# leejaeyong7/tiny-cuda-nn

Hardware: AMD Instinct MI355X
Metric: training_step throughput (samples/s) HashGrid+64-wide FFMLP, batch=256k; % fp16-MFMA peak (higher is better)
Workload: dtype f16

## Files before the change

tiny-cuda-nn_amd/csrc/capi.cpp:

```cpp
#include "../../include/tcnn_amd.h"

#include "model.h"

#include <mutex>
#include <string>

using namespace tcnn_amd;

namespace {
thread_local std::string g_last_error;
tcnn_amd::Switches g_switches;
std::mutex g_switches_mutex;

bool env_is(const char* name, char c) {
	const char* e = getenv(name);
	return e && e[0] == c;
}
int env_01(const char* name) {
	const char* e = getenv(name);
	return (e && (e[0] == '0' || e[0] == '1')) ? e[0] - '0' : -1;
}

template <typename F>
int guarded(F&& f) {
	try {
		f();
		return TCNN_OK;
	} catch (const std::exception& e) {
		g_last_error = e.what();
		log_message(TCNN_LOG_ERROR, g_last_error);
		return TCNN_ERROR;
	} catch (...) {
		g_last_error = "unknown error";
		return TCNN_ERROR;
	}
}

Json parse_or_empty(const char* text) {
	if (!text || !*text) return Json::object();
	return Json::parse(text);
}
}

struct tcnn_module_s {
	std::unique_ptr<Model> model;
	std::string hyperparams_text;
	std::string name_text;
};

struct tcnn_context_s {
	std::unique_ptr<ModelContext> ctx;
};

struct tcnn_trainer_s {
	std::unique_ptr<Trainer> trainer;
	std::string hyperparams_text;
	std::string network_hyperparams_text;
	std::vector<uint8_t> snapshot;
};

struct tcnn_train_ctx_s {
	std::unique_ptr<TrainContext> ctx;
};

struct tcnn_optimizer_s {
	std::unique_ptr<Optimizer> optimizer;
	size_t n_params = 0;
	std::string hyperparams_text;
	std::vector<uint8_t> snapshot;
};

namespace tcnn_amd {
Switches switches() {
	std::lock_guard<std::mutex> lock{g_switches_mutex};
	return g_switches;
}
void switches_reload() {
	Switches w;
	w.grid_planes = !env_is("TCNN_AMD_GRID_PLANES", '0');
	w.grid_rows_planes = !env_is("TCNN_AMD_GRID_ROWS_PLANES", '0');
	{ const char* e = getenv("TCNN_AMD_GRID_SCATTER"); w.grid_scatter_lds = !(e && std::string{e} == "atomic"); }
	w.scatter_records = !env_is("TCNN_AMD_SCATTER_RECORDS", '0');
	w.scatter_tune = !env_is("TCNN_AMD_SCATTER_TUNE", '0');
	w.scatter_lists = env_01("TCNN_AMD_SCATTER_LISTS");
	w.scatter_wide = env_is("TCNN_AMD_SCATTER_WIDE", '1');
	w.fused_step = !env_is("TCNN_AMD_FUSED_STEP", '0');
	w.side_jobs = !env_is("TCNN_AMD_SIDE_JOBS", '0');
	w.live_image = !env_is("TCNN_AMD_LIVE_IMAGE", '0');
	w.adam_steps32 = env_is("TCNN_AMD_ADAM_STEPS32", '1');
	w.adam_in_reduce = !env_is("TCNN_AMD_ADAM_IN_REDUCE", '0');
	w.adam_prologue = !env_is("TCNN_AMD_ADAM_PROLOGUE", '0');
	w.adam_prologue_refused = env_is("TCNN_AMD_ADAM_PROLOGUE", 'r');
	w.mlp_r32 = !env_is("TCNN_AMD_MLP_R32", '0');
	w.mlp_r32a = env_01("TCNN_AMD_MLP_R32A");
	w.mlp_regs = !env_is("TCNN_AMD_MLP_REGS", '0');
	w.mlp_fast = !env_is("TCNN_AMD_MLP_FAST", '0');
	if (const char* e = getenv("TCNN_AMD_MLP_PRIO")) w.mlp_prio = (uint32_t)atoi(e);
	w.listgrad_in_mlp = !env_is("TCNN_AMD_LISTGRAD_IN_MLP", '0');
	w.mlp_layerwise = env_is("TCNN_AMD_MLP_LAYERWISE", '1');
	std::lock_guard<std::mutex> lock{g_switches_mutex};
	g_switches = w;
}
}

extern "C" {

const char* tcnn_last_error(void) { return g_last_error.c_str(); }
const char* tcnn_version(void) { return "tcnn_amd 0.1 (gfx950)"; }

uint32_t tcnn_batch_size_granularity(void) { return BATCH_SIZE_GRANULARITY; }

int tcnn_device(int* device_out) {
	return guarded([&] { HIP_CHECK_THROW(hipGetDevice(device_out)); });
}

int tcnn_set_device(int device) {
	return guarded([&] { HIP_CHECK_THROW(hipSetDevice(device)); });
}

void tcnn_free_temporary_memory(void) { Arena::instance().release_all(); }

int tcnn_gpu_malloc(size_t bytes, void** out) {
	return guarded([&] {
		CHECK_THROW(out != nullptr);
		*out = nullptr;
		if (bytes) HIP_CHECK_THROW(hipMalloc(out, bytes));
	});
}
int tcnn_gpu_free(void* ptr) {
	return guarded([&] { if (ptr) HIP_CHECK_THROW(hipFree(ptr)); });
}
int tcnn_gpu_memcpy(void* dst, const void* src, size_t bytes, int kind) {
	return guarded([&] {
		const hipMemcpyKind k = kind == TCNN_MEMCPY_HOST_TO_DEVICE ? hipMemcpyHostToDevice : kind == TCNN_MEMCPY_DEVICE_TO_HOST ? hipMemcpyDeviceToHost : hipMemcpyDeviceToDevice;
		if (bytes) HIP_CHECK_THROW(hipMemcpy(dst, src, bytes, k));
	});
}
int tcnn_gpu_memset(void* ptr, int value, size_t bytes) {
	return guarded([&] { if (bytes) HIP_CHECK_THROW(hipMemset(ptr, value, bytes)); });
}
int tcnn_stream_synchronize(tcnn_stream_t stream) {
	return guarded([&] { HIP_CHECK_THROW(hipStreamSynchronize((hipStream_t)stream)); });
}
int tcnn_generate_random_uniform(tcnn_stream_t stream, uint64_t rng_state_inc[2], size_t n, float* out, float lower, float upper) {
	return guarded([&] {
		CHECK_THROW(rng_state_inc != nullptr && (out != nullptr || n == 0));
		generate_random_uniform((hipStream_t)stream, rng_state_inc, n, out, lower, upper);
		HIP_CHECK_THROW(hipGetLastError());
	});
}
int tcnn_has_networks(void) { return 1; }
float tcnn_default_loss_scale(int precision) { return precision == TCNN_PRECISION_FP32 ? 1.0f : LOSS_SCALE_FP16; }
int tcnn_preferred_precision(void) { return TCNN_PRECISION_FP16; }

void tcnn_set_log_callback(void (*callback)(int, const char*, void*), void* user) {
	log_sink().callback = callback;
	log_sink().user = user;
}

int tcnn_create_network_with_input_encoding_precision(uint32_t n_input_dims, uint32_t n_output_dims, const char* encoding_json, const char* network_json, int precision, tcnn_module_t* out) {
	switches_reload();
	return guarded([&] {
		CHECK_THROW(out != nullptr);
		if (precision != TCNN_PRECISION_FP32 && precision != TCNN_PRECISION_FP16) throw std::runtime_error{"Unknown precision " + std::to_string(precision)};
		auto m = std::make_unique<tcnn_module_s>();
		m->model.reset(new NetworkWithInputEncoding{n_input_dims, n_output_dims, parse_or_empty(encoding_json), parse_or_empty(network_json),
		                                            precision == TCNN_PRECISION_FP32 ? Precision::Fp32 : Precision::Fp16});
		*out = m.release();
	});
}

int tcnn_create_network_with_input_encoding(uint32_t n_input_dims, uint32_t n_output_dims, const char* encoding_json, const char* network_json, tcnn_module_t* out) {
	return tcnn_create_network_with_input_encoding_precision(n_input_dims, n_output_dims, encoding_json, network_json, TCNN_PRECISION_FP16, out);
}

int tcnn_create_network_precision(uint32_t n_input_dims, uint32_t n_output_dims, const char* network_json, int precision, tcnn_module_t* out) {
	return tcnn_create_network_with_input_encoding_precision(n_input_dims, n_output_dims, "{\"otype\": \"Identity\"}", network_json, precision, out);
}

int tcnn_create_network(uint32_t n_input_dims, uint32_t n_output_dims, const char* network_json, tcnn_module_t* out) {
	return tcnn_create_network_precision(n_input_dims, n_output_dims, network_json, TCNN_PRECISION_FP16, out);
}

int tcnn_create_encoding(uint32_t n_input_dims, const char* encoding_json, int precision, tcnn_module_t* out) {
	switches_reload();
	return guarded([&] {
		CHECK_THROW(out != nullptr);
		auto m = std::make_unique<tcnn_module_s>();
		m->model.reset(new EncodingModel{n_input_dims, parse_or_empty(encoding_json), precision == TCNN_PRECISION_FP32 ? Precision::Fp32 : Precision::Fp16});
		*out = m.release();
	});
}

void tcnn_module_destroy(tcnn_module_t module) { delete module; }

int tcnn_module_inference(tcnn_module_t m, tcnn_stream_t stream, uint32_t n, const float* input, void* output, void* params) {
	return guarded([&] {
		CHECK_THROW(m && m->model);
		m->model->inference((hipStream_t)stream, n, MatView{input, m->model->input_width(), 1u}, output, params);
	});
}

int tcnn_module_forward(tcnn_module_t m, tcnn_stream_t stream, uint32_t n, const float* input, void* output, void* params, int prepare_input_gradients, tcnn_context_t* ctx_out) {
	return guarded([&] {
		CHECK_THROW(m && m->model && ctx_out);
		auto c = std::make_unique<tcnn_context_s>();
		c->ctx = m->model->forward((hipStream_t)stream, n, MatView{input, m->model->input_width(), 1u}, output, params, prepare_input_gradients != 0);
		*ctx_out = c.release();
	});
}

int tcnn_module_backward(tcnn_module_t m, tcnn_stream_t stream, tcnn_context_t ctx, uint32_t n, float* dL_dinput, const void* dL_doutput, void* dL_dparams,
                         const float* input, const void* output, const void* params) {
	return guarded([&] {
		CHECK_THROW(m && m->model);
		if (!ctx || !ctx->ctx) throw std::runtime_error{"Module::bwd: called with invalid context. fwd likely (mistakenly) ran in inference mode."};
		MatViewMut dx{dL_dinput, m->model->input_width(), 1u};
		m->model->backward((hipStream_t)stream, *ctx->ctx, n, MatView{input, m->model->input_width(), 1u}, output, dL_doutput, dL_dinput ? &dx : nullptr, params,
		                   dL_dparams, dL_dparams ? GradientMode::Overwrite : GradientMode::Ignore);
	});
}

int tcnn_module_backward_backward_input(tcnn_module_t m, tcnn_stream_t stream, tcnn_context_t ctx, uint32_t n, const float* dL_ddLdinput, const float* input, const void* dL_doutput,
                                        void* dL_dparams, void* dL_ddLdoutput, float* dL_dinput, const void* params) {
	return tcnn_module_backward_backward_input_mode(m, stream, ctx, n, dL_ddLdinput, input, dL_doutput, dL_dparams, dL_ddLdoutput, dL_dinput, params,
	                                                dL_dparams ? TCNN_GRADIENT_OVERWRITE : TCNN_GRADIENT_IGNORE);
}

int tcnn_module_backward_backward_input_mode(tcnn_module_t m, tcnn_stream_t stream, tcnn_context_t ctx, uint32_t n, const float* dL_ddLdinput, const float* input, const void* dL_doutput,
                                             void* dL_dparams, void* dL_ddLdoutput, float* dL_dinput, const void* params, int gradient_mode) {
	return guarded([&] {
		CHECK_THROW(gradient_mode == TCNN_GRADIENT_IGNORE || ((gradient_mode == TCNN_GRADIENT_OVERWRITE || gradient_mode == TCNN_GRADIENT_ACCUMULATE) && dL_dparams != nullptr));
		CHECK_THROW(m && m->model);
		if (!ctx || !ctx->ctx) throw std::runtime_error{"Module::bwd_bwd_input: called with invalid context. fwd likely (mistakenly) ran in inference mode."};
		CHECK_THROW(dL_ddLdinput != nullptr && input != nullptr);
		const uint32_t w = m->model->input_width();
		MatViewMut dx{dL_dinput, w, 1u};
		m->model->backward_backward_input((hipStream_t)stream, *ctx->ctx, n, MatView{input, w, 1u}, MatView{dL_ddLdinput, w, 1u}, dL_doutput, dL_ddLdoutput, dL_dinput ? &dx : nullptr, params,
		                                  gradient_mode == TCNN_GRADIENT_IGNORE ? nullptr : dL_dparams, (GradientMode)gradient_mode);
	});
}

void tcnn_context_destroy(tcnn_context_t ctx) { delete ctx; }

uint32_t tcnn_module_n_input_dims(tcnn_module_t m) { return m->model->input_width(); }
uint32_t tcnn_module_n_output_dims(tcnn_module_t m) { return m->model->padded_output_width(); }
size_t tcnn_module_n_params(tcnn_module_t m) { return m->model->n_params(); }
size_t tcnn_module_list_scatters(tcnn_module_t m) { return (size_t)m->model->list_scatters(); }

namespace {
[[noreturn]] void no_grid(Model& model) {
	throw std::runtime_error{"max_level: " + model.name() + " has no grid encoding (GridEncoding::set_max_level, grid_interface.h:101-123)"};
}
}

int tcnn_module_set_max_level(tcnn_module_t m, float max_level) {
	return guarded([&] {
		CHECK_THROW(m && m->model);
		if (!m->model->set_max_level(max_level)) no_grid(*m->model);
	});
}
int tcnn_module_set_max_level_gpu(tcnn_module_t m, const float* per_sample) {
	return guarded([&] {
		CHECK_THROW(m && m->model);
		if (!m->model->set_max_level_gpu(per_sample)) no_grid(*m->model);
	});
}
float tcnn_module_max_level(tcnn_module_t m) {
	float v = std::numeric_limits<float>::quiet_NaN();
	const float* per_sample = nullptr;
	guarded([&] {
		CHECK_THROW(m && m->model);
		if (!m->model->get_max_level(v, per_sample)) no_grid(*m->model);
		g_last_error.clear();
	});
	return v;
}
int tcnn_module_param_precision(tcnn_module_t m) { return (int)m->model->precision(); }
int tcnn_module_output_precision(tcnn_module_t m) { return (int)m->model->precision(); }

int tcnn_module_initialize_params(tcnn_module_t m, uint64_t seed, float* params_full_precision, float scale) {
	return guarded([&] {
		CHECK_THROW(m && m->model);
		Pcg32 rng{seed};
		m->model->initialize_params(rng, params_full_precision, scale);
		HIP_CHECK_THROW(hipDeviceSynchronize());
	});
}

const char* tcnn_module_hyperparams(tcnn_module_t m) {
	m->hyperparams_text = m->model->hyperparams().dump();
	return m->hyperparams_text.c_str();
}

const char* tcnn_module_name(tcnn_module_t m) {
	m->name_text = m->model->name();
	return m->name_text.c_str();
}

int tcnn_create_from_config_precision(uint32_t n_input_dims, uint32_t n_output_dims, const char* config_json, uint32_t seed, int precision, tcnn_trainer_t* out) {
	switches_reload();
	return guarded([&] {
		CHECK_THROW(out != nullptr);
		if (precision != TCNN_PRECISION_FP32 && precision != TCNN_PRECISION_FP16) throw std::runtime_error{"Unknown precision " + std::to_string(precision)};
		auto t = std::make_unique<tcnn_trainer_s>();
		t->trainer.reset(new Trainer{n_input_dims, n_output_dims, parse_or_empty(config_json), seed, precision == TCNN_PRECISION_FP32 ? Precision::Fp32 : Precision::Fp16});
		*out = t.release();
	});
}

int tcnn_create_from_config_seeded(uint32_t n_input_dims, uint32_t n_output_dims, const char* config_json, uint32_t seed, tcnn_trainer_t* out) {
	return tcnn_create_from_config_precision(n_input_dims, n_output_dims, config_json, seed, TCNN_PRECISION_FP16, out);
}

int tcnn_trainer_precision(tcnn_trainer_t t) {
	int v = -1;
	guarded([&] { CHECK_THROW(t && t->trainer); v = (int)t->trainer->precision(); });
	return v;
}

int tcnn_create_from_config(uint32_t n_input_dims, uint32_t n_output_dims, const char* config_json, tcnn_trainer_t* out) {
	return tcnn_create_from_config_seeded(n_input_dims, n_output_dims, config_json, 1337, out);
}

void tcnn_trainer_destroy(tcnn_trainer_t t) { delete t; }

int tcnn_trainer_training_step(tcnn_trainer_t t, tcnn_stream_t stream, uint32_t n, const float* input, int input_layout, const float* target, const float* data_pdf,
                               int run_optimizer, float* dL_dinput, int use_inference_params, int gradient_mode, const void* external_dL_dy, tcnn_train_ctx_t* ctx_out) {
	return guarded([&] {
		CHECK_THROW(t && t->trainer && ctx_out);
		Trainer& tr = *t->trainer;
		const uint32_t w = tr.model().input_width();
		MatViewMut dx = make_view_mut(dL_dinput, w, n, input_layout);
		auto c = std::make_unique<tcnn_train_ctx_s>();
		c->ctx = tr.training_step((hipStream_t)stream, n, make_view(input, w, n, input_layout), target, data_pdf, run_optimizer != 0, dL_dinput ? &dx : nullptr,
		                          use_inference_params != 0, (GradientMode)gradient_mode, external_dL_dy);
		*ctx_out = c.release();
	});
}

int tcnn_trainer_loss(tcnn_trainer_t t, tcnn_stream_t stream, tcnn_train_ctx_t ctx, float* loss_out) {
	return guarded([&] {
		CHECK_THROW(t && t->trainer && ctx && ctx->ctx && loss_out);
		*loss_out = t->trainer->loss((hipStream_t)stream, *ctx->ctx);
	});
}

int tcnn_trainer_forward(tcnn_trainer_t t, tcnn_stream_t stream, float loss_scale, uint32_t n, const float* input, int input_layout, const float* target, const float* data_pdf,
                         int use_inference_params, int prepare_input_gradients, const void* external_dL_dy, tcnn_train_ctx_t* ctx_out) {
	return guarded([&] {
		CHECK_THROW(t && t->trainer && ctx_out);
		Trainer& tr = *t->trainer;
		auto c = std::make_unique<tcnn_train_ctx_s>();
		c->ctx = tr.forward((hipStream_t)stream, loss_scale, n, make_view(input, tr.model().input_width(), n, input_layout), target, data_pdf, use_inference_params != 0,
		                    prepare_input_gradients != 0, external_dL_dy);
		*ctx_out = c.release();
	});
}

int tcnn_trainer_backward(tcnn_trainer_t t, tcnn_stream_t stream, tcnn_train_ctx_t ctx, uint32_t n, const float* input, int input_layout, float* dL_dinput,
                          int use_inference_params, int gradient_mode) {
	return guarded([&] {
		CHECK_THROW(t && t->trainer && ctx && ctx->ctx);
		Trainer& tr = *t->trainer;
		const uint32_t w = tr.model().input_width();
		MatViewMut dx = make_view_mut(dL_dinput, w, n, input_layout);
		tr.backward((hipStream_t)stream, *ctx->ctx, n, make_view(input, w, n, input_layout), dL_dinput ? &dx : nullptr, use_inference_params != 0, (GradientMode)gradient_mode);
	});
}

int tcnn_trainer_optimizer_step(tcnn_trainer_t t, tcnn_stream_t stream, float loss_scale) {
	return guarded([&] {
		CHECK_THROW(t && t->trainer);
		t->trainer->optimizer_step((hipStream_t)stream, loss_scale);
	});
}

void tcnn_train_ctx_destroy(tcnn_train_ctx_t ctx) { delete ctx; }
const void* tcnn_train_ctx_output(tcnn_train_ctx_t ctx) { return ctx->ctx->output.data(); }
const void* tcnn_train_ctx_dL_doutput(tcnn_train_ctx_t ctx) {
	if (guarded([&] { ctx->ctx->materialize(); }) != 0) return nullptr;
	return ctx->ctx->dL_doutput_ptr;
}
const float* tcnn_train_ctx_L(tcnn_train_ctx_t ctx) {
	if (guarded([&] { ctx->ctx->materialize(); }) != 0) return nullptr;
	return ctx->ctx->L.as<float>();
}

int tcnn_trainer_inference(tcnn_trainer_t t, tcnn_stream_t stream, uint32_t n, const float* input, int input_layout, float* output, int output_layout, int use_inference_params) {
	return guarded([&] {
		CHECK_THROW(t && t->trainer);
		Trainer& tr = *t->trainer;
		tr.inference((hipStream_t)stream, n, make_view(input, tr.model().input_width(), n, input_layout), make_view_mut(output, tr.model().output_width(), n, output_layout),
		             use_inference_params != 0);
	});
}

int tcnn_trainer_inference_mixed_precision(tcnn_trainer_t t, tcnn_stream_t stream, uint32_t n, const float* input, int input_layout, void* output_half, int use_inference_params) {
	return guarded([&] {
		CHECK_THROW(t && t->trainer && (output_half || n == 0));
		Trainer& tr = *t->trainer;
		tr.inference_mixed_precision((hipStream_t)stream, n, make_view(input, tr.model().input_width(), n, input_layout), output_half, use_inference_params != 0);
// ... 232 lines not shown
```

tiny-cuda-nn_amd/csrc/grid_device.h:

```cpp
#pragma once

#include "tcnn_common.h"

#include <hip/hip_fp16.h>

namespace tcnn_amd {
namespace {

typedef _Float16 half_t;

template <typename T, int N> struct VecOf { typedef T type __attribute__((ext_vector_type(N))); };
template <typename T> struct VecOf<T, 1> { typedef T type; };

__device__ inline float smoothstep(float v) { return v * v * (3.0f - 2.0f * v); }
__device__ inline float smoothstep_derivative(float v) { return 6 * v * (1.0f - v); }

__device__ inline uint32_t pos_fract(float input, float scale, uint32_t interpolation, float* pos, float* pos_derivative) {
	float p = fmaf(scale, input, 0.5f);
	const float tmp = floorf(p);
	const uint32_t cell = (uint32_t)(int)tmp;
	p -= tmp;
	if (interpolation == (uint32_t)InterpolationType::Smoothstep) {
		*pos_derivative = smoothstep_derivative(p);
		*pos = smoothstep(p);
	} else {
		*pos_derivative = 1.0f;
		*pos = p;
	}
	return cell;
}

__device__ inline uint32_t rng_hash_device(const uint32_t* pos, int n_dims) {
	const uint64_t MULT = 0x5851f42d4c957f2dULL;
	const uint32_t bits_per_dim = 64 / n_dims;
	uint64_t step = 0;
	for (int i = 0; i < n_dims; ++i) step ^= (uint64_t)pos[i] << (i * bits_per_dim);
	uint64_t inc = (1ull << 1u) | 1u;
	uint64_t state = 0;
	state = state * MULT + inc;
	state += 1337ull;
	state = state * MULT + inc;
	uint64_t cur_mult = MULT, cur_plus = inc, acc_mult = 1u, acc_plus = 0u;
	uint64_t delta = step;
	while (delta > 0) {
		if (delta & 1) {
			acc_mult *= cur_mult;
			acc_plus = acc_plus * cur_mult + cur_plus;
		}
		cur_plus = (cur_mult + 1) * cur_plus;
		cur_mult *= cur_mult;
		delta /= 2;
	}
	state = acc_mult * state + acc_plus;
	const uint64_t old = state;
	const uint32_t xorshifted = (uint32_t)(((old >> 18u) ^ old) >> 27u);
	const uint32_t rot = (uint32_t)(old >> 59u);
	return (xorshifted >> rot) | (xorshifted << ((~rot + 1u) & 31));
}

template <int D, bool RNG = true>
__device__ inline uint32_t level_index(const GridLevel& lv, const uint32_t* primes, uint32_t hash_type, const uint32_t* cell) {
	uint32_t index;
	if (lv.hashed) {
		if (RNG && hash_type == (uint32_t)HashType::Rng) {
			index = rng_hash_device(cell, D);
		} else {
			index = 0;
#pragma unroll
			for (int d = 0; d < D; ++d) index ^= cell[d] * primes[d];
		}
	} else {
		index = 0;
#pragma unroll
		for (int d = 0; d < D; ++d) index += cell[d] * lv.stride[d];
	}
	if (lv.size_mask) return index & lv.size_mask;
	return index >= lv.size ? index % lv.size : index;
}

template <int D>
__device__ inline void load_coords(const MatView& x, uint32_t i, float (&out)[D]) {
	if (x.stride_dim == 1 && x.stride_sample == D && (D == 2 || D == 4)) {
		typedef float vecD __attribute__((ext_vector_type(D)));
		const vecD v = *(const vecD*)(x.data + (size_t)i * D);
#pragma unroll
		for (int d = 0; d < D; ++d) out[d] = v[d];
	} else {
#pragma unroll
		for (int d = 0; d < D; ++d) out[d] = x.data[(size_t)i * x.stride_sample + (size_t)d * x.stride_dim];
	}
}

__device__ inline uint32_t scatter_chunk(const GridLevel& lv, uint32_t index) {
	return lv.scatter_shift != 0xffffffffu ? (index >> lv.scatter_shift) : (index / lv.scatter_per_chunk);
}

}
}
```

tiny-cuda-nn_amd/csrc/k_grid_planes.hip:

```cpp
#include "grid_device.h"
#include "mlp_side_jobs.h"

#include <algorithm>
#include <cstdio>
#include <cstdlib>
#include <vector>

namespace tcnn_amd {
namespace {

constexpr int FP_THREADS = 128;
#ifndef TCNN_FP_LIST_THREADS
#define TCNN_FP_LIST_THREADS 256
#endif
constexpr int FP_LIST_THREADS = TCNN_FP_LIST_THREADS;

constexpr int FP_MAX_CHUNKS = GRID_FILTER_MAX_CHUNKS;
constexpr int FP_PER_LANE = FP_MAX_CHUNKS / 64;

template <int D, int F, int FP_SPT, bool LISTS>
__global__ void __launch_bounds__(LISTS ? FP_LIST_THREADS : FP_THREADS) k_grid_fwd_planes(
	const GridMeta* __restrict__ meta, const uint32_t* __restrict__ work, const uint32_t max_items, const uint32_t blocks_per_xcd, const uint32_t n, const MatView x,
	const half_t* __restrict__ grid, half_t* __restrict__ out, unsigned long long* __restrict__ bits, const MlpPrepJob prep, const GridHitLists lists
) {
	typedef typename VecOf<half_t, F>::type vecF;
	constexpr int THREADS = LISTS ? FP_LIST_THREADS : FP_THREADS;
	if (prep.image) {
		const uint32_t total = (prep.desc.n_frags_fwd + prep.desc.n_frags_bwd + prep.desc.n_frags_r32) * 512;
		for (uint32_t e = blockIdx.x * THREADS + threadIdx.x; e < total; e += gridDim.x * THREADS) mlp_prep_element(prep.desc, (const half_t*)prep.params, (half_t*)prep.image, e);
	}
	constexpr int FP_WAVE_SAMPLES = 64 * FP_SPT;
	constexpr int FP_ITEM_SAMPLES = THREADS * FP_SPT;
	constexpr int STAGE_ELEMS = FP_ITEM_SAMPLES << (D - 1);
	constexpr int STAGE_U64 = STAGE_ELEMS * (int)GRID_HIT_WORDS / 2 + STAGE_ELEMS / 4;
	static_assert(!LISTS || FP_ITEM_SAMPLES <= 65536, "16-bit sample numbers inside an item");
	__shared__ __attribute__((aligned(16))) unsigned long long lds_raw[LISTS ? STAGE_U64 + 72 : (FP_THREADS / 64) * FP_SPT * FP_MAX_CHUNKS];
	typedef unsigned long long plane_row[FP_SPT][FP_MAX_CHUNKS];
	plane_row* planes = (plane_row*)lds_raw;
	typedef __attribute__((address_space(3))) uint32_t lds_u32;
	uint32_t* l_stage = (uint32_t*)lds_raw;
	uint16_t* l_sidx = (uint16_t*)(lds_raw + STAGE_ELEMS * (int)GRID_HIT_WORDS / 2);
	uint32_t* l_cnt = (uint32_t*)(lds_raw + STAGE_U64);
	uint32_t* l_off = l_cnt + 64;
	uint32_t* l_total = l_cnt + 128;
	static_assert(FP_MAX_CHUNKS == 64, "one lane per chunk");
	if constexpr (LISTS) {
		if (threadIdx.x < 64) l_cnt[threadIdx.x] = 0;
		if (blockIdx.x == gridDim.x - 1 && lists.zero_counts) {
			for (uint32_t e = threadIdx.x; e < meta->n_levels * GRID_HIT_COUNT_STRIDE; e += THREADS) lists.zero_counts[e] = 0;
		}
		__syncthreads();
	}

	const uint32_t tid = threadIdx.x;
	const uint32_t lane = tid & 63;
	const uint32_t wave = __builtin_amdgcn_readfirstlane(tid >> 6);
	const uint32_t xcd = blockIdx.x & 7u, slot = blockIdx.x >> 3;
	const uint32_t n_items = work[xcd];
	const uint32_t* __restrict__ items = work + 8 + (size_t)xcd * max_items;

	const uint32_t interpolation = meta->interpolation;
	const uint32_t hash_type = meta->hash_type;
	uint32_t primes[D];
#pragma unroll
	for (int d = 0; d < D; ++d) primes[d] = meta->primes[d];
	const uint32_t n_words = n / 64;
	constexpr int C = 1 << D;
	constexpr int R_ROWS = C / 2;
	constexpr uint32_t HIT_SHIFT = grid_hit_mask_shift(D);

	for (uint32_t it = slot; it < n_items; it += blocks_per_xcd) {
		const uint32_t w = items[it];
		const uint32_t level = w >> 24;
		uint32_t base = (w & 0xffffffu) * FP_ITEM_SAMPLES + wave * FP_WAVE_SAMPLES;
		if constexpr (LISTS) base = grid_item_sample(lists.map, w & 0xffffffu, wave * FP_WAVE_SAMPLES);
		if constexpr (!LISTS) { if (base >= n) continue; }
		const GridLevel lv = meta->levels[level];
		const half_t* __restrict__ lgrid = grid + (size_t)lv.offset * F;
		half_t* __restrict__ lout = out + (size_t)level * n * F;
		const uint32_t n_chunks = lv.scatter_n_chunks;
		const bool want_bits = !LISTS && bits != nullptr && n_chunks > 1 && n_chunks <= FP_MAX_CHUNKS;
		const bool lds_or = want_bits && n_chunks > 8;
		const bool want_lists = LISTS && n_chunks > 1 && n_chunks <= FP_MAX_CHUNKS;
		uint32_t cr[FP_SPT][R_ROWS];
		uint32_t ipair[FP_SPT][R_ROWS];
		const bool nearest = interpolation == (uint32_t)InterpolationType::Nearest;

		if (lds_or) {
#pragma unroll
			for (int k = 0; k < FP_SPT; ++k)
#pragma unroll
				for (int j = 0; j < FP_PER_LANE; ++j) planes[wave][k][lane + 64 * j] = 0ull;
		}

		constexpr int R = C / 2;
		typedef typename VecOf<half_t, 2 * F>::type vecP __attribute__((aligned(2 * F)));
		vecP P[FP_SPT][R];
		vecF E[FP_SPT][R];
		uint32_t sel[FP_SPT];
		float pos[FP_SPT][D];
		unsigned long long touched[FP_SPT];
		auto note_chunk = [&](const int k, const uint32_t index) {
			const uint32_t ch = scatter_chunk(lv, index);
			if (lds_or) {
				__hip_atomic_fetch_or((__attribute__((address_space(3))) uint32_t*)&planes[wave][k][ch] + (lane >> 5), 1u << (lane & 31), __ATOMIC_RELAXED,
				                      __HIP_MEMORY_SCOPE_WAVEFRONT);
			} else {
				touched[k] |= 1ull << ch;
			}
		};
#pragma unroll
		for (int k = 0; k < FP_SPT; ++k) {
			const uint32_t i = min(base + k * 64 + lane, n - 1);
			float xin[D];
			load_coords<D>(x, i, xin);
			uint32_t cell[D];
			float pd;
#pragma unroll
			for (int d = 0; d < D; ++d) cell[d] = pos_fract(xin[d], lv.scale, interpolation, &pos[k][d], &pd);
			touched[k] = 0;
			sel[k] = 0;
			if constexpr (LISTS) {
#pragma unroll
				for (int r = 0; r < R_ROWS; ++r) { cr[k][r] = 0xffffffffu; ipair[k][r] = 0; }
			}
			const bool lists_here = LISTS && want_lists && base + k * 64 + lane < n;
#pragma unroll
			for (int r = 0; r < R; ++r) {
				if (r > 0 && nearest) { P[k][r] = P[k][0]; E[k][r] = E[k][0]; continue; }
				uint32_t local[D];
				local[0] = cell[0];
#pragma unroll
				for (int d = 1; d < D; ++d) local[d] = cell[d] + ((r >> (d - 1)) & 1);
				const uint32_t idx0 = level_index<D>(lv, primes, hash_type, local);
				local[0] = cell[0] + 1;
				const uint32_t idx1 = nearest ? idx0 : level_index<D>(lv, primes, hash_type, local);
				const uint32_t a0 = lv.hashed ? (idx0 & ~1u) : min(idx0, lv.size - 2u);
				P[k][r] = *(const vecP*)&lgrid[(size_t)a0 * F];
				const uint32_t d1 = idx1 - a0;
				const bool own = d1 > 1u;
				vecF e;
#pragma unroll
				for (int f = 0; f < F; ++f) { if constexpr (F == 1) e = (half_t)0.0f; else e[f] = (half_t)0.0f; }
				if (own) e = *(const vecF*)&lgrid[(size_t)idx1 * F];
				E[k][r] = e;
				sel[k] |= ((idx0 - a0) | ((d1 & 1u) << 1) | (own ? 4u : 0u)) << (3 * r);
				if (want_bits) {
					note_chunk(k, idx0);
					if (!nearest) note_chunk(k, idx1);
				}
				if constexpr (LISTS) {
					if (lists_here) {
						const uint32_t ch_a = scatter_chunk(lv, idx0), first = ch_a * lv.scatter_per_chunk;
						uint32_t rel_b = idx0 - first;
						if (!nearest) {
							const uint32_t ch_b = scatter_chunk(lv, idx1);
							if (ch_b == ch_a) rel_b = idx1 - first;
							else {
								const uint32_t at = atomicAdd(&lists.counts[level * GRID_HIT_COUNT_STRIDE], 1u);
								if (at < lists.straggler_capacity) {
									typedef uint32_t u2 __attribute__((ext_vector_type(2)));
									*(u2*)&lists.stragglers[((size_t)level * lists.straggler_capacity + at) * 2] = u2{i | (2u << (2 * r)) << HIT_SHIFT, ch_b};
								}
							}
						}
						ipair[k][r] = (idx0 - first) | rel_b << 16;
						const uint32_t rank = __hip_atomic_fetch_add((lds_u32*)&l_cnt[ch_a], 1u, __ATOMIC_RELAXED, __HIP_MEMORY_SCOPE_WORKGROUP);
						cr[k][r] = ch_a << 16 | rank;
					}
				}
			}
		}
		if constexpr (LISTS) {
			if (want_lists) {
				__syncthreads();
				if (wave == 0) {
					const uint32_t cnt = l_cnt[lane];
					l_cnt[lane] = 0;
					uint32_t incl = cnt;
#pragma unroll
					for (int o = 1; o < 64; o <<= 1) {
						const uint32_t up = __shfl_up(incl, o);
						if (lane >= (uint32_t)o) incl += up;
					}
					l_off[lane] = incl - cnt;
					uint32_t* heads = lists.heads + (size_t)level * GRID_HIT_HEADS * lists.n_items + (w & 0xffffffu);
#ifdef TCNN_AMD_DEV
					if (!(lists.dev_flags & 4u))
#endif
					heads[(size_t)lane * lists.n_items] = incl - cnt;
					if (lane == 63) { heads[(size_t)64 * lists.n_items] = incl; *l_total = incl; }
				}
				__syncthreads();
			}
		}

#pragma unroll
		for (int k = 0; k < FP_SPT; ++k) {
			const uint32_t i = base + k * 64 + lane;
			vecF v[C];
#pragma unroll
			for (int r = 0; r < R; ++r) {
				const uint32_t s = sel[k] >> (3 * r);
				vecF lo, hi;
#pragma unroll
				for (int f = 0; f < F; ++f) { lo[f] = P[k][r][f]; hi[f] = P[k][r][F + f]; }
				v[2 * r] = (s & 1u) ? hi : lo;
				v[2 * r + 1] = (s & 4u) ? E[k][r] : ((s & 2u) ? hi : lo);
			}
			half_t acc[F];
			half_t whs[C];
#pragma unroll
			for (int idx = 0; idx < C; ++idx) whs[idx] = (half_t)1.0f;
			if (nearest) {
#pragma unroll
				for (int f = 0; f < F; ++f) acc[f] = v[0][f];
			} else {
#pragma unroll
				for (int f = 0; f < F; ++f) acc[f] = (half_t)0.0f;
#pragma unroll
				for (int idx = 0; idx < C; ++idx) {
					float weight = 1;
#pragma unroll
					for (int d = 0; d < D; ++d) weight *= (idx & (1 << d)) == 0 ? 1 - pos[k][d] : pos[k][d];
					asm volatile("" : "+v"(weight));
					const half_t wh = (half_t)weight;
					whs[idx] = wh;
#pragma unroll
					for (int f = 0; f < F; ++f) {
						half_t val;
						val = v[idx][f];
						acc[f] = __builtin_fmaf16(wh, val, acc[f]);
					}
				}
			}
			if (base + k * 64 < n) {
				vecF o;
#pragma unroll
				for (int f = 0; f < F; ++f) { if constexpr (F == 1) o = acc[f]; else o[f] = acc[f]; }
				*(vecF*)&lout[(size_t)i * F] = o;
			}
			if constexpr (LISTS) {
				if (want_lists) {
#pragma unroll
					for (int r = 0; r < R_ROWS; ++r) {
						const uint32_t v = cr[k][r];
						if (v != 0xffffffffu) {
							const uint32_t at = l_off[v >> 16] + (v & 0xffffu);
							typedef uint32_t u2 __attribute__((ext_vector_type(2)));
							const uint32_t pr = ipair[k][r];
							const bool no_b = (pr >> 16) == (pr & 0xffffu);
							*(u2*)(l_stage + at * GRID_HIT_WORDS) = u2{pr, (uint32_t)__builtin_bit_cast(uint16_t, whs[2 * r]) | (no_b ? 0u : (uint32_t)__builtin_bit_cast(uint16_t, whs[2 * r + 1]) << 16)};
							l_sidx[at] = (uint16_t)(wave * FP_WAVE_SAMPLES + k * 64 + lane);
						}
					}
				}
			}
		}

		if constexpr (LISTS) {
			if (want_lists) {
				__syncthreads();
				typedef uint32_t u4 __attribute__((ext_vector_type(4)));
				const uint32_t total = *l_total, quads = (total * GRID_HIT_WORDS + 3) / 4, squads = (total + 7) / 8;
				const size_t region = ((size_t)level * lists.n_items + (w & 0xffffffu)) * lists.item_capacity;
				u4* dst = (u4*)(lists.elems + region * GRID_HIT_WORDS);
				u4* sdst = (u4*)(lists.sidx + region);
#ifdef TCNN_AMD_DEV
				if (!(lists.dev_flags & 1u))
#endif
				{
#ifdef TCNN_AMD_DEV
					if (lists.dev_flags & 8u) {
						const auto rs_e = __builtin_amdgcn_make_buffer_rsrc((void*)dst, 0, (int)(quads * 16u), 0x00020000);
						const auto rs_s = __builtin_amdgcn_make_buffer_rsrc((void*)sdst, 0, (int)(squads * 16u), 0x00020000);
						for (uint32_t p = tid; p < quads; p += THREADS) __builtin_amdgcn_raw_buffer_store_b128(((const u4*)l_stage)[p], rs_e, p * 16u, 0, 16);
						for (uint32_t p = tid; p < squads; p += THREADS) __builtin_amdgcn_raw_buffer_store_b128(((const u4*)l_sidx)[p], rs_s, p * 16u, 0, 16);
					} else
#endif
					{
					for (uint32_t p = tid; p < quads; p += THREADS) dst[p] = ((const u4*)l_stage)[p];
					for (uint32_t p = tid; p < squads; p += THREADS) sdst[p] = ((const u4*)l_sidx)[p];
					}
				}
			}
		}
		if (want_bits) {
#pragma unroll
			for (int j = 0; j < FP_PER_LANE; ++j) {
				if (j > 0 && !lds_or) break;
				unsigned long long mine[FP_SPT];
				const uint32_t ch = lane + 64 * j;
				if (lds_or) {
					__builtin_amdgcn_wave_barrier();
#pragma unroll
					for (int k = 0; k < FP_SPT; ++k) mine[k] = planes[wave][k][ch];
				} else {
#pragma unroll
					for (int k = 0; k < FP_SPT; ++k) {
						mine[k] = 0;
						for (uint32_t c = 0; c < n_chunks; ++c) {
							const unsigned long long b = __ballot((touched[k] >> c) & 1ull);
							if (lane == c) mine[k] = b;
						}
					}
				}
				if (ch < n_chunks) {
					unsigned long long* dst = bits + ((size_t)level * FP_MAX_CHUNKS + ch) * n_words + base / 64;
					if (base + FP_WAVE_SAMPLES <= n) {
						typedef unsigned long long u64x2 __attribute__((ext_vector_type(2)));
#pragma unroll
						for (int k = 0; k < FP_SPT; k += 2) *(u64x2*)&dst[k] = u64x2{mine[k], mine[k + 1]};
					} else {
#pragma unroll
						for (int k = 0; k < FP_SPT; ++k) if (base + k * 64 < n) dst[k] = mine[k];
					}
				}
			}
		}
	}
}

template <int D, int F, int SPT>
void launch_planes(hipStream_t s, const GridMeta* dm, const uint32_t* work, uint32_t max_items, uint32_t blocks_per_xcd, uint32_t n, MatView x, const void* grid, void* out, uint64_t* bits,
                   const MlpPrepJob* prep_job, const GridHitLists* hit_lists) {
	MlpPrepJob prep{};
	if (prep_job) prep = *prep_job;
	if (hit_lists) {
		if constexpr (SPT == 8) throw std::runtime_error{"grid_forward_planes: hit lists come from the 2- and 4-samples-per-thread shapes"};
		else
		hipLaunchKernelGGL((k_grid_fwd_planes<D, F, SPT, true>), dim3(8 * blocks_per_xcd), dim3(FP_LIST_THREADS), 0, s, dm, work, max_items, blocks_per_xcd, n, x, (const half_t*)grid, (half_t*)out,
		                   nullptr, prep, *hit_lists);
	} else {
		hipLaunchKernelGGL((k_grid_fwd_planes<D, F, SPT, false>), dim3(8 * blocks_per_xcd), dim3(FP_THREADS), 0, s, dm, work, max_items, blocks_per_xcd, n, x, (const half_t*)grid, (half_t*)out,
		                   (unsigned long long*)bits, prep, GridHitLists{});
	}
	HIP_CHECK_THROW(hipGetLastError());
}

uint32_t max_scatter_chunks(const GridMeta& meta) {
	uint32_t m = 1;
	for (uint32_t l = 0; l < meta.n_levels; ++l) m = std::max(m, meta.levels[l].scatter_n_chunks);
	return m;
}

}

uint32_t grid_hit_item_samples(const GridMeta& meta) { return FP_LIST_THREADS * grid_planes_spt(meta); }

uint32_t grid_planes_spt(const GridMeta& meta) {
	uint32_t forced = 0;
#ifdef TCNN_AMD_DEV
	static const uint32_t dev_forced = getenv("TCNN_AMD_FWD_SPT") ? (uint32_t)atoi(getenv("TCNN_AMD_FWD_SPT")) : 0u;
	forced = dev_forced;
#endif
	if (max_scatter_chunks(meta) > (uint32_t)FP_MAX_CHUNKS) return 2u;
	if (forced == 8 || forced == 4 || forced == 2) return forced;
	if (meta.n_pos_dims == 3 && grid_scatter_prefers_lists(meta)) return 2u;
	return 4u;
}

bool grid_planes_supported(const GridMeta& meta, uint32_t n) {
	const uint32_t F = meta.n_features_per_level;
	return (F == 2 || F == 4 || F == 8) && (meta.n_pos_dims == 2 || meta.n_pos_dims == 3) && meta.n_levels < 256 && n % 64 == 0 && n > 0 &&
	       div_round_up(n, FP_THREADS * grid_planes_spt(meta)) < (1u << 24);
}

void grid_planes_plan(const GridMeta& meta, uint32_t n, bool hit_lists, std::vector<uint32_t>& work, uint32_t& max_items, uint32_t& blocks_per_xcd) {
	const uint32_t threads = hit_lists ? FP_LIST_THREADS : FP_THREADS;
	const uint32_t items_per_level = div_round_up(n, threads * grid_planes_spt(meta));
	float coarse_cost = 0.6f;
#ifdef TCNN_AMD_DEV
	if (const char* e = getenv("TCNN_AMD_FWD_COARSE_COST")) coarse_cost = (float)atof(e);
#endif
	std::vector<float> cost(meta.n_levels);
	double total = 0;
	for (uint32_t l = 0; l < meta.n_levels; ++l) {
		const size_t bytes = (size_t)meta.levels[l].size * meta.n_features_per_level * 2;
		cost[l] = bytes > (256u << 10) ? 1.0f : coarse_cost;
		total += (double)cost[l] * items_per_level;
	}
	uint32_t dbg_lo = 0, dbg_hi = meta.n_levels;
#ifdef TCNN_AMD_DEV
	if (const char* e = getenv("TCNN_AMD_FWD_LEVELS")) sscanf(e, "%u,%u", &dbg_lo, &dbg_hi);
#endif
	(void)total;
	size_t wide_bytes = (size_t)4 << 20;
#ifdef TCNN_AMD_DEV
	if (const char* e = getenv("TCNN_AMD_FWD_WIDE_MB")) wide_bytes = (size_t)std::max(atoi(e), 0) << 20;
#endif
	auto is_wide = [&](uint32_t l) { return wide_bytes > 0 && (size_t)meta.levels[l].size * meta.n_features_per_level * 2 > wide_bytes; };
	double narrow_total = 0;
	for (uint32_t l = 0; l < meta.n_levels; ++l) if (l >= dbg_lo && l <= dbg_hi && !is_wide(l)) narrow_total += (double)cost[l] * items_per_level;
	std::vector<std::vector<uint32_t>> runs(8);
	double acc = 0;
	for (uint32_t l = 0; l < meta.n_levels; ++l) {
		if (l < dbg_lo || l > dbg_hi || is_wide(l)) continue;
		for (uint32_t i = 0; i < items_per_level; ++i) {
			const uint32_t bin = std::min<uint32_t>((uint32_t)((acc + 0.5 * cost[l]) * 8.0 / narrow_total), 7u);
			runs[bin].push_back(l << 24 | i);
			acc += cost[l];
		}
	}
	{
		size_t longest = 0;
		for (auto& r : runs) longest = std::max(longest, r.size());
		uint32_t next = 0;
		for (uint32_t l = 0; l < meta.n_levels; ++l) {
			if (l < dbg_lo || l > dbg_hi || !is_wide(l)) continue;
			for (uint32_t i = 0; i < items_per_level; ++i) {
				size_t best = next % 8;
				for (size_t b = 0; b < 8; ++b) if (runs[b].size() < runs[best].size()) best = b;
				runs[best].push_back(l << 24 | i);
				++next;
			}
		}
		(void)longest;
	}
	max_items = 0;
	for (auto& r : runs) max_items = std::max<uint32_t>(max_items, (uint32_t)r.size());
	work.assign(8 + (size_t)8 * max_items, 0xffffffffu);
	for (uint32_t b = 0; b < 8; ++b) {
		work[b] = (uint32_t)runs[b].size();
		std::copy(runs[b].begin(), runs[b].end(), work.begin() + 8 + (size_t)b * max_items);
	}
	blocks_per_xcd = std::max(1u, std::min(256u * FP_THREADS / threads, max_items));
#ifdef TCNN_AMD_DEV
	if (const char* e = getenv("TCNN_AMD_FWD_BLOCKS_PER_XCD")) blocks_per_xcd = std::max(1, atoi(e));
#endif
}

void grid_forward_planes(hipStream_t stream, const GridMeta& meta, const GridMeta* dev_meta, const uint32_t* dev_work, uint32_t max_items, uint32_t blocks_per_xcd, uint32_t n,
                         MatView x, const void* grid, void* out_planes, uint64_t* chunk_bits, const MlpPrepJob* prep_job, const GridHitLists* hit_lists) {
	CHECK_THROW(grid_planes_supported(meta, n));
	CHECK_THROW(!hit_lists || (hit_lists->elems && hit_lists->heads && hit_lists->stragglers && hit_lists->counts && n <= grid_hit_max_samples(meta) &&
	                           hit_lists->item_samples == grid_hit_item_samples(meta) && hit_lists->n_items == div_round_up(n, hit_lists->item_samples) &&
	                           hit_lists->sidx && hit_lists->item_capacity >= (hit_lists->item_samples << (meta.n_pos_dims - 1)) && hit_lists->item_capacity % 8 == 0));
	if (hit_lists) {
		const GridItemMap& m = hit_lists->map;
		CHECK_THROW(m.window > 0 && m.window == (1u << m.window_shift) && m.window * m.n_windows == hit_lists->item_samples && m.window % (64 * grid_planes_spt(meta)) == 0);
		CHECK_THROW(m.n_windows == 1 || (n % hit_lists->item_samples == 0 && m.stride == hit_lists->n_items * m.window));
	}
	const uint32_t F = meta.n_features_per_level;
#define TCNN_PLANES_F(D, SPT) \
	switch (F) { \
		case 2: return launch_planes<D, 2, SPT>(stream, dev_meta, dev_work, max_items, blocks_per_xcd, n, x, grid, out_planes, chunk_bits, prep_job, hit_lists); \
		case 4: return launch_planes<D, 4, SPT>(stream, dev_meta, dev_work, max_items, blocks_per_xcd, n, x, grid, out_planes, chunk_bits, prep_job, hit_lists); \
		default: return launch_planes<D, 8, SPT>(stream, dev_meta, dev_work, max_items, blocks_per_xcd, n, x, grid, out_planes, chunk_bits, prep_job, hit_lists); \
	}
#define TCNN_PLANES(D) \
	if (grid_planes_spt(meta) == 8) { TCNN_PLANES_F(D, 8) } else if (grid_planes_spt(meta) == 4) { TCNN_PLANES_F(D, 4) } else { TCNN_PLANES_F(D, 2) }
	if (meta.n_pos_dims == 2) { TCNN_PLANES(2) } else { TCNN_PLANES(3) }
#undef TCNN_PLANES
#undef TCNN_PLANES_F
}

namespace {
constexpr uint32_t PR_THREADS = 256, PR_SAMPLES = 64, PR_MAX_WORDS = 128;
__global__ void __launch_bounds__(PR_THREADS) k_planes_to_rows(const uint32_t* __restrict__ planes, uint32_t* __restrict__ rows, const uint32_t n, const uint32_t words_per_level,
                                                                const uint32_t words, const uint32_t row_words) {
	__shared__ uint32_t tile[PR_SAMPLES * (PR_MAX_WORDS + 1)];
	const uint32_t i0 = blockIdx.x * PR_SAMPLES, pitch = words + 1;
	const uint32_t per_level = PR_SAMPLES * words_per_level;
	for (uint32_t idx = threadIdx.x; idx < PR_SAMPLES * words; idx += PR_THREADS) {
		const uint32_t l = idx / per_level, r = idx - l * per_level;
		const uint32_t i = r / words_per_level, k = r - i * words_per_level;
		tile[i * pitch + l * words_per_level + k] = planes[((size_t)l * n + i0) * words_per_level + r];
	}
	__syncthreads();
	for (uint32_t idx = threadIdx.x; idx < PR_SAMPLES * words; idx += PR_THREADS) {
		const uint32_t i = idx / words, w = idx - i * words;
		rows[(size_t)(i0 + i) * row_words + w] = tile[i * pitch + w];
	}
}
__global__ void __launch_bounds__(PR_THREADS) k_rows_to_planes(const uint32_t* __restrict__ rows, uint32_t* __restrict__ planes, const uint32_t n, const uint32_t words_per_level,
                                                                const uint32_t words, const uint32_t row_words) {
	__shared__ uint32_t tile[PR_SAMPLES * (PR_MAX_WORDS + 1)];
	const uint32_t i0 = blockIdx.x * PR_SAMPLES, pitch = words + 1;
	const uint32_t per_level = PR_SAMPLES * words_per_level;
	for (uint32_t idx = threadIdx.x; idx < PR_SAMPLES * words; idx += PR_THREADS) {
		const uint32_t i = idx / words, w = idx - i * words;
		tile[i * pitch + w] = rows[(size_t)(i0 + i) * row_words + w];
	}
	__syncthreads();
	for (uint32_t idx = threadIdx.x; idx < PR_SAMPLES * words; idx += PR_THREADS) {
		const uint32_t l = idx / per_level, r = idx - l * per_level;
		const uint32_t i = r / words_per_level, k = r - i * words_per_level;
		planes[((size_t)l * n + i0) * words_per_level + r] = tile[i * pitch + l * words_per_level + k];
	}
}
}

bool grid_planes_to_rows_supported(const GridMeta& meta, uint32_t n, uint32_t width) {
	const uint32_t F = meta.n_features_per_level;
	return n > 0 && n % PR_SAMPLES == 0 && F % 2 == 0 && width > 0 && width % F == 0 && width / 2 <= PR_MAX_WORDS;
}

void grid_planes_to_rows(hipStream_t stream, const GridMeta& meta, uint32_t n, uint32_t width, const void* planes, void* rows, uint32_t row_stride) {
	CHECK_THROW(grid_planes_to_rows_supported(meta, n, width) && row_stride % 2 == 0 && row_stride >= width);
	hipLaunchKernelGGL(k_planes_to_rows, dim3(n / PR_SAMPLES), dim3(PR_THREADS), 0, stream, (const uint32_t*)planes, (uint32_t*)rows, n, meta.n_features_per_level / 2, width / 2, row_stride / 2);
}

void grid_rows_to_planes(hipStream_t stream, const GridMeta& meta, uint32_t n, uint32_t width, const void* rows, uint32_t row_stride, void* planes) {
	CHECK_THROW(grid_planes_to_rows_supported(meta, n, width) && row_stride % 2 == 0 && row_stride >= width);
	hipLaunchKernelGGL(k_rows_to_planes, dim3(n / PR_SAMPLES), dim3(PR_THREADS), 0, stream, (const uint32_t*)rows, (uint32_t*)planes, n, meta.n_features_per_level / 2, width / 2, row_stride / 2);
}

}
```

tiny-cuda-nn_amd/csrc/model.h:

```cpp
#pragma once

#include "json_lite.h"
#include "tcnn_common.h"
#include "mlp_side_jobs.h"

#include <algorithm>
#include <cctype>
#include <cstdio>
#include <cmath>
#include <cstring>
#include <functional>
#include <limits>
#include <map>
#include <memory>
#include <mutex>
#include <numeric>
#include <random>
#include <unordered_map>
#include <vector>

namespace tcnn_amd {

struct LogSink {
	void (*callback)(int, const char*, void*) = nullptr;
// ... 98 lines not shown
	size_t bytes() const { return m_bytes; }
	explicit operator bool() const { return m_ptr != nullptr; }
private:
	void* m_ptr = nullptr;
	hipStream_t m_stream = nullptr;
	size_t m_bytes = 0, m_capacity = 0;
	int m_dev = 0;
};

class DeviceBuf {
public:
	DeviceBuf() = default;
	explicit DeviceBuf(size_t bytes) { resize(bytes); }
	~DeviceBuf() { if (m_ptr) (void)hipFree(m_ptr); }
	DeviceBuf(const DeviceBuf&) = delete;
	DeviceBuf& operator=(const DeviceBuf&) = delete;
	DeviceBuf(DeviceBuf&& o) noexcept : m_ptr{o.m_ptr}, m_bytes{o.m_bytes} { o.m_ptr = nullptr; o.m_bytes = 0; }
	DeviceBuf& operator=(DeviceBuf&& o) noexcept {
		if (this != &o) {
			if (m_ptr) (void)hipFree(m_ptr);
			m_ptr = o.m_ptr; m_bytes = o.m_bytes;
			o.m_ptr = nullptr; o.m_bytes = 0;
		}
		return *this;
	}
	void resize(size_t bytes) {
		if (bytes == m_bytes) return;
		if (m_ptr) { (void)hipFree(m_ptr); m_ptr = nullptr; }
		m_bytes = bytes;
		if (bytes) HIP_CHECK_THROW(hipMalloc(&m_ptr, bytes));
	}
	void memset(int v) { if (m_bytes) HIP_CHECK_THROW(hipMemset(m_ptr, v, m_bytes)); }
	void* data() const { return m_ptr; }
	template <typename T> T* as() const { return (T*)m_ptr; }
	size_t bytes() const { return m_bytes; }
private:
	void* m_ptr = nullptr;
	size_t m_bytes = 0;
};

struct Pcg32 {
	uint64_t st[2] = {0x853c49e6748fea9bULL, 0xda3e39cb94b95bdbULL};
	static constexpr uint64_t MULT = 0x5851f42d4c957f2dULL;
	Pcg32() = default;
	explicit Pcg32(uint64_t initstate, uint64_t initseq = 1) {
		st[0] = 0;
		st[1] = (initseq << 1u) | 1u;
		next_uint();
		st[0] += initstate;
		next_uint();
	}
	uint32_t next_uint() {
		const uint64_t old = st[0];
		st[0] = old * MULT + st[1];
		const uint32_t xorshifted = (uint32_t)(((old >> 18u) ^ old) >> 27u);
		const uint32_t rot = (uint32_t)(old >> 59u);
		return (xorshifted >> rot) | (xorshifted << ((~rot + 1u) & 31));
	}
	float next_float() {
		const uint32_t u = (next_uint() >> 9) | 0x3f800000u;
		float f;
		memcpy(&f, &u, 4);
		return f - 1.0f;
	}
};

struct EncodingContext {
	ArenaBuf to_reduce;
	ArenaBuf dy_dx;
	ArenaBuf chunk_mask;
	ArenaBuf hit_elems;
	GridHitLists hit_lists;
	uint64_t hit_generation = 0;
	const void* hit_stream = nullptr;
	uint32_t n = 0;
	GridForwardRoute route;
	std::vector<EncodingContext> nested;
};

struct BackwardHandoff {
	const MlpReduceJob* reduce_job = nullptr;
	AdamPrologue* prologue = nullptr;
	void* list_gradients = nullptr;
	bool reduce_carried = false;
};

struct ForwardPlan {
	GridForwardRoute route;
	const MlpPrepJob* prep_job = nullptr;
	const GridItemMap* item_map = nullptr;
};

class Encoding {
public:
	virtual ~Encoding() {}
	virtual uint32_t input_width() const = 0;
	virtual uint32_t output_width() const = 0;
	uint32_t padded_output_width() const { return output_width() + m_n_to_pad; }
	virtual uint32_t required_output_alignment() const { return 1; }
	virtual void set_padded_output_width(uint32_t padded) {
		CHECK_THROW(padded >= output_width());
		m_n_to_pad = padded - output_width();
	}
	void set_alignment(uint32_t alignment) {
		const uint32_t a = std::lcm(alignment, required_output_alignment());
		set_padded_output_width(next_multiple(output_width(), a));
	}
	virtual size_t n_params() const { return 0; }
	virtual void initialize_params(Pcg32& rng, float* params_full_precision, float scale) {}
	virtual EncodingContext forward(hipStream_t stream, uint32_t n, MatView x, const void* params, void* out, bool prepare_input_gradients, bool prepare_param_gradients, const ForwardPlan* plan = nullptr) = 0;
	virtual void backward(hipStream_t stream, const EncodingContext& ctx, uint32_t n, MatView x, const void* dL_dy, MatViewMut* dL_dx, const void* params, void* grads, GradientMode mode, const GridBackwardRoute& route, BackwardHandoff* handoff = nullptr) = 0;
	virtual GridBackwardRoute backward_route(const Switches& sw, hipStream_t stream, const EncodingContext& ctx, uint32_t n, MatView x, GridDyForm offer, bool want_dL_dx, GradientMode mode) { return {}; }
	void backward_rows(hipStream_t stream, const EncodingContext& ctx, uint32_t n, MatView x, const void* dL_dy, MatViewMut* dL_dx, const void* params, void* grads, GradientMode mode) {
		backward(stream, ctx, n, x, dL_dy, dL_dx, params, grads, mode, backward_route(switches(), stream, ctx, n, x, GridDyForm::Rows, dL_dx != nullptr, mode));
	}
	virtual void backward_backward_input(hipStream_t stream, const EncodingContext& ctx, uint32_t n, MatView x, MatView dL_ddLdx, const void* dL_dy, void* dL_ddLdy,
	                                     MatViewMut* dL_dx, const void* params, void* grads, GradientMode mode) {
		throw std::runtime_error{"DifferentiableObject::backward_backward_input_impl: not implemented error"};
	}
	virtual bool has_second_order() const { return false; }
	virtual bool second_order_reads_dL_dy() const { return true; }
	virtual bool as_identity(float& scale, float& offset) const { return false; }
	virtual uint32_t as_oneblob() const { return 0; }
	virtual uint64_t scatter_wide_fallbacks() { return 0; }
	virtual uint64_t list_scatters() const { return 0; }
	virtual GridForwardRoute forward_route(const Switches& sw, uint32_t n, bool as_planes, bool prepare_input_gradients, bool prepare_param_gradients) const { return {}; }
	virtual Json hyperparams() const = 0;
	bool fp32() const { return m_fp32; }
	virtual bool set_max_level(float max_level) { return false; }
	virtual bool set_max_level_gpu(const float* per_sample) { return false; }
	virtual bool get_max_level(float& max_level, const float*& per_sample) const { return false; }
protected:
	explicit Encoding(bool fp32) : m_fp32{fp32} {}
	bool m_fp32;
	uint32_t m_n_to_pad = 0;
};

inline GridType string_to_grid_type(const std::string& s) {
	if (equals_case_insensitive(s, "Hash")) return GridType::Hash;
	if (equals_case_insensitive(s, "Dense")) return GridType::Dense;
	if (equals_case_insensitive(s, "Tiled") || equals_case_insensitive(s, "Tile")) return GridType::Tiled;
	throw std::runtime_error{"Invalid grid type: " + s};
}
inline HashType string_to_hash_type(const std::string& s) {
	if (equals_case_insensitive(s, "Prime")) return HashType::Prime;
	if (equals_case_insensitive(s, "CoherentPrime")) return HashType::CoherentPrime;
	if (equals_case_insensitive(s, "ReversedPrime")) return HashType::ReversedPrime;
	if (equals_case_insensitive(s, "Rng")) return HashType::Rng;
	throw std::runtime_error{"Invalid hash type: " + s};
}
inline InterpolationType string_to_interpolation_type(const std::string& s) {
	if (equals_case_insensitive(s, "Nearest")) return InterpolationType::Nearest;
	if (equals_case_insensitive(s, "Linear")) return InterpolationType::Linear;
	if (equals_case_insensitive(s, "Smoothstep")) return InterpolationType::Smoothstep;
	throw std::runtime_error{"Invalid interpolation type: " + s};
}

class GridEncoding : public Encoding {
public:
	GridEncoding(uint32_t n_dims_to_encode, const Json& enc, bool fp32) : Encoding{fp32} {
		const uint32_t F = enc.value("n_features_per_level", 2u);
		if (F != 1 && F != 2 && F != 4 && F != 8) throw std::runtime_error{"GridEncoding: n_features_per_level must be 1, 2, 4, or 8."};
		const uint32_t log2_hashmap_size = enc.value("log2_hashmap_size", 19u);
		const std::string encoding_type = enc.value("otype", "Grid");
		const std::string default_type = equals_case_insensitive(encoding_type, "TiledGrid") ? "Tiled" : (equals_case_insensitive(encoding_type, "DenseGrid") ? "Dense" : "Hash");
		uint32_t n_features;
		if (enc.contains("n_features") || enc.contains("n_grid_features")) {
			n_features = enc.contains("n_features") ? enc.value("n_features", 0u) : enc.value("n_grid_features", 0u);
			if (enc.contains("n_levels")) throw std::runtime_error{"GridEncoding: may not specify n_features and n_levels simultaneously (one determines the other)"};
		} else {
			n_features = F * enc.value("n_levels", 16u);
		}
		const uint32_t n_levels = n_features / F;
		const GridType grid_type = string_to_grid_type(enc.value("type", default_type));
		const uint32_t base_resolution = enc.value("base_resolution", 16u);
		const float per_level_scale = enc.value("per_level_scale", grid_type == GridType::Dense ? std::exp(std::log(256.0f / (float)base_resolution) / (n_levels - 1)) : 2.0f);
		const HashType hash_type = string_to_hash_type(enc.value("hash", "CoherentPrime"));
		m_stochastic_interpolation = enc.value("stochastic_interpolation", false);
		if (m_stochastic_interpolation) throw std::runtime_error{"GridEncoding: stochastic_interpolation is not supported by this build"};
		if (n_dims_to_encode < 2 || n_dims_to_encode > 4) throw std::runtime_error{"GridEncoding: number of input dims must be 2 or 3."};
		if (n_levels > MAX_N_LEVELS) throw std::runtime_error{"GridEncoding: m_n_levels must be at most MAX_N_LEVELS=128"};
		if (n_features % F != 0) throw std::runtime_error{"GridEncoding: n_features must be a multiple of N_FEATURES_PER_LEVEL"};

		m_n_features = n_features;
		m_log2_hashmap_size = log2_hashmap_size;
		m_base_resolution = base_resolution;
		m_per_level_scale = per_level_scale;

		memset(&m_meta, 0, sizeof(m_meta));
		m_meta.n_pos_dims = n_dims_to_encode;
		m_meta.n_features_per_level = F;
		m_meta.n_levels = n_levels;
		m_meta.grid_type = (uint32_t)grid_type;
		m_meta.hash_type = (uint32_t)hash_type;
		m_meta.interpolation = (uint32_t)string_to_interpolation_type(enc.value("interpolation", "Linear"));
		static const uint32_t prime[7] = {1958374283u, 2654435761u, 805459861u, 3674653429u, 2097192037u, 1434869437u, 2165219737u};
		static const uint32_t coherent[7] = {1u, 2654435761u, 805459861u, 3674653429u, 2097192037u, 1434869437u, 2165219737u};
		static const uint32_t reversed[7] = {2165219737u, 1434869437u, 2097192037u, 3674653429u, 805459861u, 2654435761u, 1958374283u};
		const uint32_t* primes = hash_type == HashType::Prime ? prime : (hash_type == HashType::ReversedPrime ? reversed : coherent);
		for (uint32_t d = 0; d < 4; ++d) m_meta.primes[d] = primes[d];

		const float log2_scale = std::log2(per_level_scale);
		uint32_t offset = 0;
		for (uint32_t i = 0; i < n_levels; ++i) {
			const float scale = exp2f(i * log2_scale) * base_resolution - 1.0f;
			const uint32_t resolution = (uint32_t)ceilf(scale) + 1;
			const uint32_t max_params = std::numeric_limits<uint32_t>::max() / 2;
			uint32_t params_in_level = std::pow((float)resolution, n_dims_to_encode) > (float)max_params ? max_params : powi(resolution, n_dims_to_encode);
			params_in_level = next_multiple(params_in_level, 8u);
			if (grid_type == GridType::Tiled) params_in_level = std::min(params_in_level, powi(base_resolution, n_dims_to_encode));
			else if (grid_type == GridType::Hash) params_in_level = std::min(params_in_level, 1u << log2_hashmap_size);

			GridLevel& lv = m_meta.levels[i];
			lv.offset = offset;
			lv.size = params_in_level;
			lv.scale = scale;
			uint32_t stride = 1;
			for (uint32_t d = 0; d < 4; ++d) lv.stride[d] = 0;
			for (uint32_t d = 0; d < n_dims_to_encode && stride <= params_in_level; ++d) {
				lv.stride[d] = stride;
				stride *= resolution;
			}
			lv.hashed = (grid_type == GridType::Hash && params_in_level < stride) ? 1u : 0u;
			lv.size_mask = (params_in_level & (params_in_level - 1)) == 0 ? params_in_level - 1 : 0;
			m_resolutions.push_back(resolution);
			offset += params_in_level;
		}
		m_n_entries = offset;
		m_n_params = (size_t)offset * F;
		if (F >= 2) {
			grid_scatter_setup_levels(m_meta);
			for (uint32_t i = 0; i < n_levels; ++i) {
				m_scatter_levels_ok &= m_meta.levels[i].scatter_binned || m_meta.levels[i].scatter_n_chunks <= grid_scatter_max_chunks();
				m_any_binned |= m_meta.levels[i].scatter_binned != 0;
			}
		}
	}

	const GridMeta* dev_meta() {
		if (!m_dev_meta.data()) {
			m_dev_meta.resize(sizeof(GridMeta));
			HIP_CHECK_THROW(hipMemcpy(m_dev_meta.data(), &m_meta, sizeof(GridMeta), hipMemcpyHostToDevice));
		}
		return (const GridMeta*)m_dev_meta.data();
	}

	static uint32_t powi(uint32_t base, uint32_t exponent) {
		uint32_t result = 1;
		for (uint32_t i = 0; i < exponent; ++i) result *= base;
		return result;
	}

	uint32_t input_width() const override { return m_meta.n_pos_dims; }
	uint32_t output_width() const override { return m_n_features; }
	uint32_t required_output_alignment() const override { return m_meta.n_features_per_level; }
	size_t n_params() const override { return m_n_params; }
	const GridMeta& meta() const { return m_meta; }
	const std::vector<uint32_t>& resolutions() const { return m_resolutions; }

	void initialize_params(Pcg32& rng, float* params_full_precision, float scale) override {
		generate_random_uniform(nullptr, rng.st, n_params(), params_full_precision, -1e-4f * scale, 1e-4f * scale);
	}

	EncodingContext forward(hipStream_t stream, uint32_t n, MatView x, const void* params, void* out, bool prepare_input_gradients, bool prepare_param_gradients, const ForwardPlan* plan) override {
		EncodingContext ctx;
		if ((!out && !prepare_input_gradients) || padded_output_width() == 0 || n == 0) return ctx;
		const GridForwardRoute route = plan ? plan->route : forward_route(switches(), n, false, prepare_input_gradients, prepare_param_gradients);
		if (route.kernel == GridForwardKernel::Planes) return forward_planes(stream, route, n, x, params, out, plan->prep_job, plan->item_map);
		if (route.kernel == GridForwardKernel::PlanesToRows) {
			ArenaBuf planes{stream, (size_t)n * padded_output_width() * sizeof(uint16_t)};
			ctx = forward_planes(stream, route, n, x, params, planes.data());
			grid_planes_to_rows(stream, m_meta, n, padded_output_width(), planes.data(), out, padded_output_width());
			return ctx;
		}
		ctx.route = route;
		if (prepare_input_gradients) ctx.dy_dx = ArenaBuf{stream, (size_t)n * m_n_features * m_meta.n_pos_dims * sizeof(float)};
		const bool want_filter = route.recorded == GridRecorded::BitPlanes;
		ArenaBuf mask;
		if (want_filter) mask = ArenaBuf{stream, (size_t)m_meta.n_levels * n * (GRID_FILTER_MAX_CHUNKS / 64) * sizeof(uint64_t)};
		grid_forward(stream, m_meta, dev_meta(), m_fp32, n, x, params, out, padded_output_width(), ctx.dy_dx.as<float>(), mask.as<uint64_t>());
		if (max_level_forward_active()) {
			const uint32_t F = m_meta.n_features_per_level, D = m_meta.n_pos_dims;
			if (out) zero_levels(stream, m_fp32 ? 4 : 2, n, F, padded_output_width(), F, out, false);
			if (ctx.dy_dx) zero_levels(stream, 4, n, F * D, (uint64_t)m_n_features * D, (uint64_t)F * D, ctx.dy_dx.data(), false);
		}
		if (want_filter) {
			ctx.chunk_mask = ArenaBuf{stream, (size_t)m_meta.n_levels * grid_scatter_max_chunks() * (n / 64) * sizeof(uint64_t)};
			ctx.n = n;
			grid_mask_to_bits(stream, m_meta, dev_meta(), n, mask.as<uint64_t>(), ctx.chunk_mask.as<uint64_t>());
		}
		return ctx;
	}

	GridFacts facts() const { return GridFacts{&m_meta, m_fp32, m_scatter_levels_ok, m_any_binned, m_n_to_pad}; }
	GridForwardRoute forward_route(const Switches& sw, uint32_t n, bool as_planes, bool prepare_input_gradients, bool prepare_param_gradients) const override {
		return grid_forward_route(facts(), sw, n, as_planes, prepare_input_gradients, prepare_param_gradients);
	}

	struct PlanesPlan {
		DeviceBuf dev_work;
		uint32_t max_items = 0, blocks_per_xcd = 0;
	};
	PlanesPlan& planes_plan(uint32_t n_, bool hit_lists) {
		const uint32_t n = n_ | (hit_lists ? 0x80000000u : 0u);
		auto it = m_planes_plans.find(n);
		if (it != m_planes_plans.end()) return *it->second;
		auto plan = std::make_unique<PlanesPlan>();
		std::vector<uint32_t> work;
		grid_planes_plan(m_meta, n_, hit_lists, work, plan->max_items, plan->blocks_per_xcd);
		plan->dev_work.resize(work.size() * sizeof(uint32_t));
		HIP_CHECK_THROW(hipMemcpy(plan->dev_work.data(), work.data(), work.size() * sizeof(uint32_t), hipMemcpyHostToDevice));
		return *(m_planes_plans[n] = std::move(plan));
	}

	EncodingContext forward_planes(hipStream_t stream, const GridForwardRoute& route, uint32_t n, MatView x, const void* params, void* out_planes,
	                               const MlpPrepJob* prep_job = nullptr, const GridItemMap* item_map = nullptr) {
		EncodingContext ctx;
		CHECK_THROW(route.planned && route.kernel != GridForwardKernel::Rows);
		ctx.route = route;
		const bool want_lists = route.recorded == GridRecorded::HitLists;
		if (want_lists) {
			HitCounters& hc = hit_counters(stream);
			GridHitLists& hl = ctx.hit_lists;
			hl.item_samples = grid_hit_item_samples(m_meta);
			hl.n_items = div_round_up(n, hl.item_samples);
			hl.item_capacity = hl.item_samples << (m_meta.n_pos_dims - 1);
			hl.straggler_capacity = n << (m_meta.n_pos_dims - 1);
			hl.map = grid_item_map(hl.item_samples, 0, 1);
			if (item_map && item_map->n_windows > 1 && item_map->window * item_map->n_windows == hl.item_samples && n % hl.item_samples == 0 &&
			    item_map->stride == hl.n_items * item_map->window && item_map->window % (64 * grid_planes_spt(m_meta)) == 0) hl.map = *item_map;
			const size_t L = m_meta.n_levels;
			const size_t elems_bytes = L * hl.n_items * hl.item_capacity * GRID_HIT_WORDS * sizeof(uint32_t), sidx_bytes = next_multiple_sz(L * hl.n_items * hl.item_capacity * sizeof(uint16_t), 256);
			const size_t heads_bytes = next_multiple_sz(L * hl.n_items * GRID_HIT_HEADS * sizeof(uint32_t), 256);
			ctx.hit_elems = ArenaBuf{stream, elems_bytes + sidx_bytes + heads_bytes + L * hl.straggler_capacity * 2 * sizeof(uint32_t)};
			hl.elems = ctx.hit_elems.as<uint32_t>();
			hl.sidx = (uint16_t*)((char*)ctx.hit_elems.data() + elems_bytes);
			hl.heads = (uint32_t*)((char*)ctx.hit_elems.data() + elems_bytes + sidx_bytes);
			hl.stragglers = (uint32_t*)((char*)ctx.hit_elems.data() + elems_bytes + sidx_bytes + heads_bytes);
			hl.counts = hc.sets[hc.next].as<uint32_t>();
			hl.zero_counts = hc.sets[hc.next ^ 1].as<uint32_t>();
			hc.next ^= 1;
#ifdef TCNN_AMD_DEV
			if (const char* e = getenv("TCNN_AMD_FWD_LISTS_DEV")) hl.dev_flags = (uint32_t)atoi(e);
#endif
			ctx.hit_generation = ++hc.generation;
			ctx.hit_stream = (const void*)stream;
			ctx.n = n;
		} else if (route.recorded == GridRecorded::BitPlanes) {
			ctx.chunk_mask = ArenaBuf{stream, (size_t)m_meta.n_levels * grid_scatter_max_chunks() * (n / 64) * sizeof(uint64_t)};
			ctx.n = n;
		}
		PlanesPlan& plan = planes_plan(n, want_lists);
		grid_forward_planes(stream, m_meta, dev_meta(), plan.dev_work.as<uint32_t>(), plan.max_items, plan.blocks_per_xcd, n, x, params, out_planes, ctx.chunk_mask.as<uint64_t>(), prep_job,
		                    want_lists ? &ctx.hit_lists : nullptr);
		if (m_n_to_pad) HIP_CHECK_THROW(hipMemsetAsync((uint16_t*)out_planes + (size_t)n * m_n_features, 0, (size_t)n * m_n_to_pad * sizeof(uint16_t), stream));
		if (max_level_forward_active()) {
			const uint32_t F = m_meta.n_features_per_level;
			zero_levels(stream, 2, n, F, F, (uint64_t)n * F, out_planes, false);
		}
		return ctx;
	}

	bool lists_current(hipStream_t stream, const EncodingContext& ctx, uint32_t n) { return ctx.hit_elems && ctx.n == n && ctx.hit_stream == (const void*)stream && hit_counters(stream).generation == ctx.hit_generation; }
	GridMaxLevel max_level_state() const { return m_max_level_gpu ? GridMaxLevel::PerSample : (levels_on(true) < m_meta.n_levels ? GridMaxLevel::Scalar : GridMaxLevel::None); }
	GridBackwardRoute backward_route(const Switches& sw, hipStream_t stream, const EncodingContext& ctx, uint32_t n, MatView x, GridDyForm offer, bool want_dL_dx, GradientMode mode) override {
		GridBackwardRoute r = grid_backward_route(facts(), sw, ctx.route, lists_current(stream, ctx, n), n, offer, want_dL_dx, mode, max_level_state(), x.stride_dim == 1 && x.stride_sample == m_meta.n_pos_dims);
		const GridHitLists& hl = ctx.hit_lists;
		r.tail = r.tail && hl.map.n_windows >= 2 && hl.n_items * hl.item_samples == n;
		if (r.tail) {
			r.list_tail.sidx = hl.sidx, r.list_tail.heads = hl.heads, r.list_tail.map = hl.map;
			r.list_tail.n_items = hl.n_items, r.list_tail.item_capacity = hl.item_capacity;
			r.tail_bytes = grid_list_gradients_bytes(m_meta, hl);
		}
		return r;
	}

	void backward(hipStream_t stream, const EncodingContext& ctx, uint32_t n, MatView x, const void* dL_dy, MatViewMut* dL_dx, const void* params, void* grads, GradientMode mode, const GridBackwardRoute& route, BackwardHandoff* handoff) override {
		if ((!dL_dx && mode == GradientMode::Ignore) || n == 0) return;
		const BackwardHandoff offer = handoff ? *handoff : BackwardHandoff{};
		const auto all_levels = [&](const void* dy) {
			const bool carried = backward_all_levels(stream, ctx, n, x, dy, dL_dx, params, grads, mode, route, offer);
			if (handoff) handoff->reduce_carried = carried;
		};
		const GridMaxLevel max_level = max_level_state();
		if (max_level == GridMaxLevel::None) return all_levels(dL_dy);
		if (max_level == GridMaxLevel::PerSample) {
			const uint32_t F = m_meta.n_features_per_level;
			const bool dy_planes = route.dy == GridDyForm::Planes;
			const size_t elem = dy_planes ? 2 : (m_fp32 ? 4 : 2);
			ArenaBuf masked{stream, (size_t)n * padded_output_width() * elem};
			zero_levels(stream, elem, n, F, dy_planes ? F : padded_output_width(), dy_planes ? (uint64_t)n * F : F, masked.data(), true, dL_dy);
			return all_levels(masked.data());
		}
		GradientTail tail{*this, stream, grads, mode, levels_on(true)};
		all_levels(dL_dy);
		tail.settle();
	}

	bool backward_all_levels(hipStream_t stream, const EncodingContext& ctx, uint32_t n, MatView x, const void* dL_dy, MatViewMut* dL_dx, const void* params, void* grads, GradientMode mode,
	                         const GridBackwardRoute& route, const BackwardHandoff& offer) {
		const uint32_t F = m_meta.n_features_per_level;
		const bool dy_planes = route.dy != GridDyForm::Rows, accumulate = mode == GradientMode::Accumulate;
		uint32_t dy_stride_sample = dy_planes ? F : padded_output_width(), dy_stride_level = dy_planes ? n * F : F;
		bool carried = false;
		if (mode != GradientMode::Ignore) CHECK_THROW(grads != nullptr && route.kernel != GridGradientKernel::None);
		switch (mode == GradientMode::Ignore ? GridGradientKernel::None : route.kernel) {
		case GridGradientKernel::None: break;
		case GridGradientKernel::AtomicScratch32: {
			ArenaBuf tmp{stream, n_params() * sizeof(float)};
			if (mode == GradientMode::Overwrite) HIP_CHECK_THROW(hipMemsetAsync(tmp.data(), 0, n_params() * sizeof(float), stream));
			else cast_half_to_float(stream, n_params(), grads, tmp.as<float>());
			grid_backward(stream, m_meta, dev_meta(), true, n, x, dL_dy, false, padded_output_width(), tmp.data());
			cast_float_to_half(stream, n_params(), tmp.as<float>(), grads);
		} break;
		case GridGradientKernel::Atomic:
			if (mode == GradientMode::Overwrite) HIP_CHECK_THROW(hipMemsetAsync(grads, 0, n_params() * (m_fp32 ? 4 : 2), stream));
			grid_backward(stream, m_meta, dev_meta(), m_fp32, n, x, dL_dy, m_fp32, padded_output_width(), grads);
			break;
		case GridGradientKernel::Lists: {
			ScatterPlan& plan = scatter_plan(n, stream, true);
			ArenaBuf dy_as_planes;
			const void* dy_src = dL_dy;
			if (!dy_planes && grid_planes_to_rows_supported(m_meta, n, m_n_features)) {
				dy_as_planes = ArenaBuf{stream, (size_t)n * m_n_features * sizeof(uint16_t)};
				grid_rows_to_planes(stream, m_meta, n, m_n_features, dL_dy, padded_output_width(), dy_as_planes.data());
				dy_src = dy_as_planes.data(), dy_stride_sample = F, dy_stride_level = n * F;
			}
			++m_list_scatters;
			const bool defer = take_prologue(route, offer, plan, grads, mode);
			const bool filled = offer.list_gradients != nullptr;
			ArenaBuf gvals;
			if (!filled) gvals = ArenaBuf{stream, grid_list_gradients_bytes(m_meta, ctx.hit_lists)};
			carried = grid_backward_lists(stream, m_meta, dev_meta(), plan.dev_tasks.as<GridScatterTask>(), plan.n_tasks, plan.dev_ranges.as<GridScatterRange>(), defer ? 0u : plan.n_ranges,
			                              plan.scratch.as<uint64_t>(), n, x, dy_src, dy_stride_sample, dy_stride_level, grads, ctx.hit_lists, filled ? offer.list_gradients : gvals.data(), accumulate,
			                              defer ? nullptr : offer.reduce_job, hit_counters(stream).fallbacks.as<uint32_t>(), filled) ||
			          (defer && offer.reduce_job);
		} break;
		case GridGradientKernel::BitPlanes: {
			ScatterPlan& plan = scatter_plan(n, stream, false);
			const uint64_t* mask = (ctx.chunk_mask && ctx.n == n) ? ctx.chunk_mask.as<uint64_t>() : nullptr;
			const bool tune = route.tune && !plan.tuned && mask && plan.n_tasks > 0 && ++plan.launches == 2;
			DeviceBuf times;
			if (tune) {
				times.resize((size_t)plan.n_tasks * 8 * sizeof(uint64_t));
				times.memset(0);
			}
			const bool defer = !tune && take_prologue(route, offer, plan, grads, mode);
			carried = grid_backward_lds(stream, m_meta, dev_meta(), plan.dev_tasks.as<GridScatterTask>(), plan.n_tasks, plan.dev_ranges.as<GridScatterRange>(), defer ? 0u : plan.n_ranges,
			                            plan.scratch.as<uint64_t>(), n, x, dL_dy, dy_stride_sample, dy_stride_level, grads, mask, accumulate, route.dy == GridDyForm::Records,
			                            tune ? times.as<uint64_t>() : nullptr, defer ? nullptr : offer.reduce_job) ||
			          (defer && offer.reduce_job);
			if (route.binned) {
				ArenaBuf workspace{stream, grid_bin_workspace_bytes(m_meta, n)};
				grid_backward_binned(stream, m_meta, dev_meta(), n, x, dL_dy, dy_stride_sample, dy_stride_level, grads, accumulate, workspace.data(), hit_counters(stream).fallbacks.as<uint32_t>());
			}
			if (tune) {
				HIP_CHECK_THROW(hipStreamSynchronize(stream));
				std::vector<uint64_t> h((size_t)plan.n_tasks * 8);
				HIP_CHECK_THROW(hipMemcpy(h.data(), times.data(), h.size() * sizeof(uint64_t), hipMemcpyDeviceToHost));
				const std::vector<float> level_us = grid_scatter_level_costs(m_meta, plan.host_tasks, h);
				build_scatter_plan(plan, n, &level_us);
				plan.tuned = true;
			}
		} break;
		}
		if (dL_dx) {
			CHECK_THROW(ctx.dy_dx);
			grid_backward_input(stream, m_meta, m_fp32, n, dL_dy, padded_output_width(), ctx.dy_dx.as<float>(), *dL_dx);
		}
		return carried;
	}

	bool has_second_order() const override { return true; }
	void backward_backward_input(hipStream_t stream, const EncodingContext& ctx, uint32_t n, MatView x, MatView dL_ddLdx, const void* dL_dy, void* dL_ddLdy,
	                             MatViewMut* dL_dx, const void* params, void* grads, GradientMode mode) override {
		if ((!dL_ddLdy && mode == GradientMode::Ignore && !dL_dx) || padded_output_width() == 0 || n == 0) return;
		const uint32_t l_bwd = m_max_level_gpu ? m_meta.n_levels : levels_on(true);
		if (!m_max_level_gpu && l_bwd == m_meta.n_levels) return backward_backward_input_all_levels(stream, ctx, n, x, dL_ddLdx, dL_dy, dL_ddLdy, dL_dx, params, grads, mode);
		ArenaBuf masked;
		if (dL_dy) {
			const uint32_t F = m_meta.n_features_per_level;
			const size_t elem = m_fp32 ? 4 : 2;
			masked = ArenaBuf{stream, (size_t)n * padded_output_width() * elem};
			zero_levels(stream, elem, n, F, padded_output_width(), F, masked.data(), true, dL_dy);
			dL_dy = masked.data();
		}
		GradientTail tail{*this, stream, grads, mode, l_bwd};
		backward_backward_input_all_levels(stream, ctx, n, x, dL_ddLdx, dL_dy, dL_ddLdy, dL_dx, params, grads, mode);
		tail.settle();
	}

	void backward_backward_input_all_levels(hipStream_t stream, const EncodingContext& ctx, uint32_t n, MatView x, MatView dL_ddLdx, const void* dL_dy, void* dL_ddLdy,
	                                        MatViewMut* dL_dx, const void* params, void* grads, GradientMode mode) {
		const size_t elem = m_fp32 ? 4 : 2;
		if (dL_ddLdy) CHECK_THROW(ctx.dy_dx);
		const float* dy_dx = ctx.dy_dx.as<float>();
		if (mode != GradientMode::Ignore) {
			CHECK_THROW(grads != nullptr);
			const bool scratch32 = !m_fp32 && m_meta.n_features_per_level == 1;
			if (scratch32) {
				ArenaBuf tmp{stream, n_params() * sizeof(float)};
				if (mode == GradientMode::Overwrite) HIP_CHECK_THROW(hipMemsetAsync(tmp.data(), 0, n_params() * sizeof(float), stream));
				else cast_half_to_float(stream, n_params(), grads, tmp.as<float>());
				grid_backward_backward_input(stream, m_meta, dev_meta(), false, true, n, x, dL_ddLdx, dL_dy, padded_output_width(), params, dy_dx, tmp.data(), nullptr, nullptr);
				cast_float_to_half(stream, n_params(), tmp.as<float>(), grads);
			} else {
				if (mode == GradientMode::Overwrite) HIP_CHECK_THROW(hipMemsetAsync(grads, 0, n_params() * elem, stream));
				grid_backward_backward_input(stream, m_meta, dev_meta(), m_fp32, m_fp32, n, x, dL_ddLdx, dL_dy, padded_output_width(), params, dy_dx, grads, nullptr, nullptr);
			}
		}
		if (dL_ddLdy || dL_dx) {
			grid_backward_backward_input(stream, m_meta, dev_meta(), m_fp32, m_fp32, n, x, dL_ddLdx, dL_dy, padded_output_width(), params, dy_dx, nullptr, dL_ddLdy, dL_dx);
		}
	}

	struct ScatterPlan {
		DeviceBuf dev_tasks, dev_ranges, scratch;
		std::vector<GridScatterTask> host_tasks;
		std::vector<GridScatterRange> host_ranges;
		uint32_t n_tasks = 0, n_ranges = 0;
		uint32_t launches = 0;
		bool lists = false;
		bool tuned = false;
	};
	bool take_prologue(const GridBackwardRoute& route, const BackwardHandoff& offer, const ScatterPlan& plan, void* grads, GradientMode mode) const {
		AdamPrologue* p = offer.prologue;
		if (!route.prologue || !p || p->pending || (plan.host_ranges.empty() && !offer.reduce_job)) return false;
		p->dev_ranges = plan.dev_ranges.as<GridScatterRange>();
		p->ranges = plan.host_ranges;
		p->scratch = plan.scratch.as<uint64_t>();
		p->grad_base = grads;
		p->accumulate = mode == GradientMode::Accumulate;
		p->has_reduce = offer.reduce_job != nullptr;
		if (offer.reduce_job) {
			p->reduce_elems = offer.reduce_job->n_elems;
			p->reduce_slabs = offer.reduce_job->n_slabs;
			p->slabs = offer.reduce_job->slabs;
			p->reduce_accumulate = offer.reduce_job->accumulate;
		}
		p->pending = true;
		return true;
	}

	void build_scatter_plan(ScatterPlan& plan, uint32_t n, const std::vector<float>* measured_level_us) {
		size_t scratch_elems = 0;
		if (plan.lists) grid_scatter_lists_plan(m_meta, n, plan.host_tasks, plan.host_ranges, scratch_elems);
		else grid_scatter_plan(m_meta, n, plan.host_tasks, plan.host_ranges, scratch_elems, measured_level_us);
		plan.n_tasks = (uint32_t)plan.host_tasks.size();
		plan.n_ranges = (uint32_t)plan.host_ranges.size();
		auto upload = [](DeviceBuf& b, const void* src, size_t bytes) {
			b.resize(bytes);
			if (bytes) HIP_CHECK_THROW(hipMemcpy(b.data(), src, bytes, hipMemcpyHostToDevice));
		};
		upload(plan.dev_tasks, plan.host_tasks.data(), plan.host_tasks.size() * sizeof(GridScatterTask));
		upload(plan.dev_ranges, plan.host_ranges.data(), plan.host_ranges.size() * sizeof(GridScatterRange));
		plan.scratch.resize(0);
		plan.scratch.resize(scratch_elems * sizeof(uint64_t));
		plan.scratch.memset(0);
	}
	ScatterPlan& scatter_plan(uint32_t n, hipStream_t stream, bool lists) {
		const auto key = std::make_pair(n | (lists ? 0x80000000u : 0u), (const void*)stream);
		auto it = m_scatter_plans.find(key);
		if (it != m_scatter_plans.end()) return *it->second;
		auto plan = std::make_unique<ScatterPlan>();
		plan->lists = lists;
		build_scatter_plan(*plan, n, nullptr);
		return *(m_scatter_plans[key] = std::move(plan));
	}

	static size_t next_multiple_sz(size_t v, size_t m) { return (v + m - 1) / m * m; }
	struct HitCounters {
		DeviceBuf sets[2], fallbacks;
		int next = 0;
		uint64_t generation = 0;
	};
	HitCounters& hit_counters(hipStream_t stream) {
		auto it = m_hit_counters.find((const void*)stream);
		if (it != m_hit_counters.end()) return *it->second;
		auto hc = std::make_unique<HitCounters>();
		for (auto& set : hc->sets) {
			set.resize((size_t)m_meta.n_levels * GRID_HIT_COUNT_STRIDE * sizeof(uint32_t));
			set.memset(0);
		}
		hc->fallbacks.resize(sizeof(uint32_t));
		hc->fallbacks.memset(0);
		return *(m_hit_counters[(const void*)stream] = std::move(hc));
	}
public:
	uint64_t scatter_wide_fallbacks() override {
		uint64_t total = 0;
		for (auto& kv : m_hit_counters) {
			uint32_t v = 0;
			HIP_CHECK_THROW(hipMemcpy(&v, kv.second->fallbacks.data(), sizeof(v), hipMemcpyDeviceToHost));
			total += v;
		}
		return total;
	}

	uint64_t list_scatters() const override { return m_list_scatters; }

	bool set_max_level(float max_level) override { m_max_level = max_level; return true; }
	bool set_max_level_gpu(const float* per_sample) override { m_max_level_gpu = per_sample; return true; }
	bool get_max_level(float& max_level, const float*& per_sample) const override {
		max_level = m_max_level;
		per_sample = m_max_level_gpu;
		return true;
	}

	uint32_t levels_on(bool gradient_rule) const {
		const volatile float m = (m_max_level * (float)m_n_features) / (float)m_meta.n_features_per_level;
		const volatile float threshold = m + 1e-3f;
		for (uint32_t l = 0; l < m_meta.n_levels; ++l) {
// ... 2903 lines not shown
```

tiny-cuda-nn_amd/csrc/tcnn_common.h:

```cpp
#pragma once

#include <hip/hip_runtime.h>

#include <cstddef>
#include <cstdint>
#include <stdexcept>
#include <string>
#include <vector>

namespace tcnn_amd {

enum class Activation : uint32_t { None = 0, ReLU = 1, LeakyReLU = 2, Exponential = 3, Sine = 4, Sigmoid = 5, Squareplus = 6, Softplus = 7, Tanh = 8 };
enum class GridType : uint32_t { Hash = 0, Dense = 1, Tiled = 2 };
enum class HashType : uint32_t { Prime = 0, CoherentPrime = 1, ReversedPrime = 2, Rng = 3 };
enum class InterpolationType : uint32_t { Nearest = 0, Linear = 1, Smoothstep = 2 };
enum class LossType : uint32_t { L2 = 0, RelativeL2 = 1, L1 = 2, RelativeL1 = 3, Mape = 4, Smape = 5, CrossEntropy = 6, Variance = 7, RelativeL2Luminance = 8 };
enum class Precision : uint32_t { Fp32 = 0, Fp16 = 1 };
enum class GradientPrecision : uint32_t { Fp32 = 0, Fp16 = 1 };
enum class GradientMode : uint32_t { Ignore = 0, Overwrite = 1, Accumulate = 2 };

constexpr uint32_t BATCH_SIZE_GRANULARITY = 256;
constexpr float LOSS_SCALE_FP16 = 128.0f;
constexpr uint32_t MAX_N_LEVELS = 128;
constexpr uint32_t MAX_MLP_LAYERS = 16;

#define TCNN_STR2(x) #x
#define TCNN_STR(x) TCNN_STR2(x)
#define CHECK_THROW(x) \
	do { if (!(x)) throw std::runtime_error{std::string{__FILE__ ":" TCNN_STR(__LINE__) " check failed: " #x}}; } while (0)
#define HIP_CHECK_THROW(x) \
	do { hipError_t _e = (x); if (_e != hipSuccess) throw std::runtime_error{std::string{__FILE__ ":" TCNN_STR(__LINE__) " " #x " failed: "} + hipGetErrorString(_e)}; } while (0)

inline uint32_t div_round_up(uint32_t v, uint32_t d) { return (v + d - 1) / d; }

struct Switches {
	bool grid_planes = true;
	bool grid_rows_planes = true;
	bool grid_scatter_lds = true;
	bool scatter_records = true;
	bool scatter_tune = true;
	int scatter_lists = -1;
	bool scatter_wide = false;
	bool fused_step = true;
	bool side_jobs = true;
	bool live_image = true;
	bool adam_steps32 = false;
	bool adam_in_reduce = true;
	bool adam_prologue = true;
	bool adam_prologue_refused = false;
	bool mlp_r32 = true;
	int mlp_r32a = -1;
	bool mlp_regs = true;
	bool mlp_fast = true;
	uint32_t mlp_prio = 1;
	bool listgrad_in_mlp = true;
	bool mlp_layerwise = false;
};
Switches switches();
void switches_reload();
inline uint32_t next_multiple(uint32_t v, uint32_t d) { return div_round_up(v, d) * d; }

struct GridLevel {
	uint32_t offset;
	uint32_t size;
	float    scale;
	uint32_t hashed;
	uint32_t stride[4];
	uint32_t size_mask;
	uint32_t scatter_per_chunk;
	uint32_t scatter_shift;
	uint32_t scatter_n_chunks;
	uint32_t scatter_binned;
};

struct GridMeta {
	uint32_t n_pos_dims;
	uint32_t n_features_per_level;
	uint32_t n_levels;
	uint32_t grid_type;
	uint32_t hash_type;
	uint32_t interpolation;
	uint32_t primes[4];
	GridLevel levels[MAX_N_LEVELS];
};

struct MatView {
	const float* data;
	uint32_t stride_sample;
	uint32_t stride_dim;
};
struct MatViewMut {
	float* data;
	uint32_t stride_sample;
	uint32_t stride_dim;
};

void grid_forward(hipStream_t stream, const GridMeta& meta, const GridMeta* dev_meta, bool fp32, uint32_t n, MatView x, const void* grid, void* out, uint32_t out_stride, float* dy_dx,
                  uint64_t* chunk_mask);
bool grid_planes_supported(const GridMeta& meta, uint32_t n);
bool grid_planes_to_rows_supported(const GridMeta& meta, uint32_t n, uint32_t width);
void grid_planes_to_rows(hipStream_t stream, const GridMeta& meta, uint32_t n, uint32_t width, const void* planes, void* rows, uint32_t row_stride);
void grid_rows_to_planes(hipStream_t stream, const GridMeta& meta, uint32_t n, uint32_t width, const void* rows, uint32_t row_stride, void* planes);
uint32_t grid_planes_spt(const GridMeta& meta);
void grid_planes_plan(const GridMeta& meta, uint32_t n, bool hit_lists, std::vector<uint32_t>& work, uint32_t& max_items, uint32_t& blocks_per_xcd);
struct MlpPrepJob;
inline constexpr uint32_t grid_hit_mask_shift(uint32_t n_pos_dims) { return 32u - (1u << n_pos_dims); }
constexpr uint32_t GRID_HIT_COUNT_STRIDE = 64;
constexpr uint32_t GRID_HIT_HEADS = 65;
constexpr uint32_t GRID_HIT_WORDS = 2;
struct GridItemMap {
	uint32_t window = 0, window_shift = 0, stride = 0, n_windows = 0;
	bool operator==(const GridItemMap& o) const { return window == o.window && window_shift == o.window_shift && stride == o.stride && n_windows == o.n_windows; }
};
inline GridItemMap grid_item_map(uint32_t window, uint32_t stride, uint32_t n_windows) {
	GridItemMap m;
	m.window = window, m.stride = stride, m.n_windows = n_windows;
	while ((1u << m.window_shift) < window) ++m.window_shift;
	return m;
}
#if defined(__HIPCC__)
__host__ __device__
#endif
inline uint32_t grid_item_sample(const GridItemMap& m, uint32_t item, uint32_t pos) { return (item << m.window_shift) + (pos & (m.window - 1u)) + (pos >> m.window_shift) * m.stride; }
struct GridHitLists {
	uint32_t* elems = nullptr;
	uint16_t* sidx = nullptr;
	uint32_t* heads = nullptr;
	uint32_t* stragglers = nullptr;
	uint32_t* counts = nullptr;
	uint32_t* zero_counts = nullptr;
	uint32_t n_items = 0, item_samples = 0, item_capacity = 0, straggler_capacity = 0;
	GridItemMap map;
	uint32_t dev_flags = 0;
};
struct GridListTail {
	const uint16_t* sidx = nullptr;
	const uint32_t* heads = nullptr;
	void* gvals = nullptr;
	uint32_t n_items = 0, item_capacity = 0, n_levels = 0, level_mask = 0;
	GridItemMap map;
};
uint32_t grid_hit_item_samples(const GridMeta& meta);
inline uint32_t grid_hit_max_samples(const GridMeta& meta) { return meta.n_pos_dims <= 2 ? (1u << 24) : (1u << 22); }
void grid_forward_planes(hipStream_t stream, const GridMeta& meta, const GridMeta* dev_meta, const uint32_t* dev_work, uint32_t max_items, uint32_t blocks_per_xcd, uint32_t n,
                         MatView x, const void* grid, void* out_planes, uint64_t* chunk_bits, const MlpPrepJob* prep_job = nullptr, const GridHitLists* hit_lists = nullptr);
void grid_backward(hipStream_t stream, const GridMeta& meta, const GridMeta* dev_meta, bool fp32_grad, uint32_t n, MatView x, const void* dL_dy, bool dy_fp32, uint32_t dy_stride, void* grad);

struct GridScatterTask {
	uint32_t level;
	uint32_t entry_begin, n_entries;
	uint32_t sample_begin, sample_end;
	uint32_t flush_atomic;
	uint32_t scratch_begin;
	uint32_t pad;
};
struct GridScatterRange { size_t grad_begin; uint32_t n_elems; uint32_t scratch_begin; uint32_t pad; };
struct MlpReduceJob;
constexpr uint32_t GRID_FILTER_MAX_CHUNKS = 64;
uint32_t grid_scatter_max_chunks();
void grid_scatter_setup_levels(GridMeta& meta);
bool grid_scatter_prefers_lists(const GridMeta& meta);
void grid_scatter_plan(const GridMeta& meta, uint32_t n, std::vector<GridScatterTask>& tasks, std::vector<GridScatterRange>& shared_ranges, size_t& scratch_elems,
                       const std::vector<float>* measured_level_us = nullptr);
std::vector<float> grid_scatter_level_costs(const GridMeta& meta, const std::vector<GridScatterTask>& tasks, const std::vector<uint64_t>& times);
void grid_mask_to_bits(hipStream_t stream, const GridMeta& meta, const GridMeta* dev_meta, uint32_t n, const uint64_t* chunk_mask, uint64_t* chunk_bits);
bool grid_backward_lds(hipStream_t stream, const GridMeta& meta, const GridMeta* dev_meta, const GridScatterTask* dev_tasks, uint32_t n_tasks,
                       const GridScatterRange* dev_ranges, uint32_t n_ranges, uint64_t* scratch, uint32_t n, MatView x,
                       const void* dL_dy, uint32_t dy_stride_sample, uint32_t dy_stride_level, void* grad, const uint64_t* chunk_bits, bool accumulate, bool dy_records = false,
                       uint64_t* task_times = nullptr,
                       const MlpReduceJob* reduce_job = nullptr);
uint32_t grid_scatter_lists_lds_bytes();
void grid_scatter_lists_plan(const GridMeta& meta, uint32_t n, std::vector<GridScatterTask>& tasks, std::vector<GridScatterRange>& shared_ranges, size_t& scratch_elems);
bool grid_backward_lists(hipStream_t stream, const GridMeta& meta, const GridMeta* dev_meta, const GridScatterTask* dev_tasks, uint32_t n_tasks,
                         const GridScatterRange* dev_ranges, uint32_t n_ranges, uint64_t* scratch, uint32_t n, MatView x,
                         const void* dL_dy, uint32_t dy_stride_sample, uint32_t dy_stride_level, void* grad, const GridHitLists& lists, void* gvals, bool accumulate,
                         const MlpReduceJob* reduce_job, uint32_t* fallback_count = nullptr, bool gvals_filled = false);
size_t grid_list_gradients_bytes(const GridMeta& meta, const GridHitLists& lists);
bool grid_scatter_finalize(hipStream_t stream, const GridScatterRange* dev_ranges, uint32_t n_ranges, uint64_t* scratch, void* grad, bool accumulate, const MlpReduceJob* reduce_job);
bool grid_scatter_records_supported(const GridMeta& meta);
uint32_t grid_scatter_record_planes(const GridMeta& meta);

struct GridFacts {
	const GridMeta* meta;
	bool fp32, scatter_levels_ok, any_binned;
	uint32_t n_to_pad;
};
enum class GridForwardKernel : uint32_t { Rows, Planes, PlanesToRows };
enum class GridRecorded : uint32_t { Nothing, BitPlanes, HitLists };
struct GridForwardRoute {
	bool planned = false;
	GridForwardKernel kernel = GridForwardKernel::Rows;
	GridRecorded recorded = GridRecorded::Nothing;
	bool lds = false;
	uint32_t plane_features = 0;
};
inline bool grid_lds_gradients(const GridFacts& g, const Switches& sw, uint32_t n) {
	return !g.fp32 && g.meta->n_features_per_level >= 2 && sw.grid_scatter_lds && g.scatter_levels_ok && n % 64 == 0;
}
inline bool grid_hit_lists_wanted(const GridFacts& g, const Switches& sw, uint32_t n) {
	const GridMeta& meta = *g.meta;
	if (sw.scatter_lists == 0) return false;
	if (g.any_binned || n > grid_hit_max_samples(meta) || meta.n_pos_dims > 3 || meta.hash_type == (uint32_t)HashType::Rng) return false;
	if (sw.scatter_lists == 1) return true;
	if (meta.n_pos_dims == 2 && n < (1u << 16)) return false;
	return grid_scatter_prefers_lists(meta);
}
inline GridForwardRoute grid_forward_route(const GridFacts& g, const Switches& sw, uint32_t n, bool as_planes, bool input_gradients, bool param_gradients) {
	const GridMeta& meta = *g.meta;
	const uint32_t F = meta.n_features_per_level;
	GridForwardRoute r;
	r.planned = true;
	r.lds = grid_lds_gradients(g, sw, n);
	const bool planes = !input_gradients && !g.fp32 && sw.grid_planes && g.n_to_pad % F == 0 && grid_planes_supported(meta, n);
	if (planes && as_planes) r.kernel = GridForwardKernel::Planes;
	else if (planes && sw.grid_rows_planes && grid_planes_to_rows_supported(meta, n, meta.n_levels * F + g.n_to_pad)) r.kernel = GridForwardKernel::PlanesToRows;
	if (r.kernel == GridForwardKernel::Planes) r.plane_features = F;
	if (param_gradients && r.lds) r.recorded = (r.kernel != GridForwardKernel::Rows && grid_hit_lists_wanted(g, sw, n)) ? GridRecorded::HitLists : GridRecorded::BitPlanes;
	return r;
}

enum class GridDyForm : uint32_t { Rows, Planes, Records };
enum class GridGradientKernel : uint32_t { None, Atomic, AtomicScratch32, BitPlanes, Lists };
enum class GridMaxLevel : uint32_t { None, Scalar, PerSample };
struct GridBackwardRoute {
	GridDyForm dy = GridDyForm::Rows;
	uint32_t plane_features = 0, record_planes = 0;
	GridGradientKernel kernel = GridGradientKernel::None;
	bool binned = false, tune = false, prologue = false;
	bool tail = false;
	GridListTail list_tail;
	size_t tail_bytes = 0;
};
inline GridBackwardRoute grid_backward_route(const GridFacts& g, const Switches& sw, const GridForwardRoute& fwd, bool lists_current, uint32_t n, GridDyForm offer, bool want_dL_dx,
                                             GradientMode mode, GridMaxLevel max_level, bool x_contiguous) {
	const GridMeta& meta = *g.meta;
	const uint32_t F = meta.n_features_per_level;
	GridBackwardRoute r;
	if (mode == GradientMode::Ignore) return r;
	if (!(fwd.planned ? fwd.lds : grid_lds_gradients(g, sw, n))) {
		r.kernel = (!g.fp32 && F == 1) ? GridGradientKernel::AtomicScratch32 : GridGradientKernel::Atomic;
		return r;
	}
	const bool lists = fwd.recorded == GridRecorded::HitLists && lists_current;
	r.kernel = lists ? GridGradientKernel::Lists : GridGradientKernel::BitPlanes;
	r.binned = !lists && g.any_binned;
	r.tune = !lists && sw.scatter_tune;
	r.prologue = max_level != GridMaxLevel::Scalar && !g.any_binned;
	if (offer == GridDyForm::Rows || want_dL_dx) return r;
	r.dy = GridDyForm::Planes, r.plane_features = F;
	if (offer == GridDyForm::Records && fwd.recorded != GridRecorded::HitLists && g.n_to_pad == 0 && max_level != GridMaxLevel::PerSample && sw.scatter_records && !g.any_binned &&
	    grid_scatter_records_supported(meta) && x_contiguous) {
		r.dy = GridDyForm::Records, r.record_planes = grid_scatter_record_planes(meta);
		return r;
	}
	r.tail = offer == GridDyForm::Records && lists && F == 2 && max_level == GridMaxLevel::None && sw.listgrad_in_mlp && meta.n_levels <= 16 &&
	         (grid_hit_item_samples(meta) << (meta.n_pos_dims - 1)) <= 2048;
	if (r.tail) {
		r.list_tail.n_levels = meta.n_levels;
		for (uint32_t l = 0; l < meta.n_levels; ++l) {
			const GridLevel& lv = meta.levels[l];
			if (lv.scatter_n_chunks > 1 && lv.scatter_n_chunks <= GRID_FILTER_MAX_CHUNKS && !lv.scatter_binned) r.list_tail.level_mask |= 1u << l;
		}
	}
	return r;
}

void ppng1_forward(hipStream_t stream, bool fp32_out, uint32_t n, uint32_t F, uint32_t Q, uint32_t C, uint32_t R, int32_t log2_min_freq, int32_t log2_max_freq, MatView x,
                   const void* features, void* out, uint32_t out_stride);
void ppng1_backward(hipStream_t stream, bool fp32_dy, uint32_t n, uint32_t F, uint32_t Q, uint32_t C, uint32_t R, int32_t log2_min_freq, int32_t log2_max_freq, MatView x,
                    const void* features, const void* dL_dy, uint32_t dy_stride, uint64_t* scratch, void* grad, bool accumulate);

void ppng2_forward(hipStream_t stream, bool fp32_out, uint32_t n, uint32_t F, uint32_t Q, uint32_t C, uint32_t R, int32_t log2_min_freq, int32_t log2_max_freq, MatView x,
                   const void* features, void* out, uint32_t out_stride);
void ppng2_backward(hipStream_t stream, bool fp32_dy, uint32_t n, uint32_t F, uint32_t Q, uint32_t C, uint32_t R, int32_t log2_min_freq, int32_t log2_max_freq, MatView x,
                    const void* features, const void* dL_dy, uint32_t dy_stride, uint64_t* scratch, void* grad, bool accumulate);
void ppng3_forward(hipStream_t stream, bool fp32_out, uint32_t n, uint32_t F, uint32_t Q, uint32_t C, int32_t log2_min_freq, int32_t log2_max_freq, MatView x, const void* features, void* out,
                   uint32_t out_stride);
size_t ppng3_backward_workspace_bytes(uint32_t n, uint32_t F, uint32_t Q, uint32_t C);
void ppng3_backward(hipStream_t stream, bool fp32_dy, uint32_t n, uint32_t F, uint32_t Q, uint32_t C, int32_t log2_min_freq, int32_t log2_max_freq, MatView x, const void* dL_dy,
                    uint32_t dy_stride, void* workspace, uint64_t* scratch, void* grad, bool accumulate);
void ppng3_backward_input(hipStream_t stream, bool fp32_dy, uint32_t n, uint32_t F, uint32_t Q, uint32_t C, int32_t log2_min_freq, int32_t log2_max_freq, MatView x, const void* features,
                          const void* dL_dy, uint32_t dy_stride, MatViewMut dL_dx);
void ppng3_backward_backward_input(hipStream_t stream, bool fp32_dy, uint32_t n, uint32_t F, uint32_t Q, uint32_t C, int32_t log2_min_freq, int32_t log2_max_freq, MatView x, MatView dL_ddLdx,
                                   const void* features, const void* dL_dy, uint32_t dy_stride, uint64_t* scratch, void* grad, bool accumulate, void* dL_ddLdy, MatViewMut* dL_dx);

bool grid_bin_supported(const GridMeta& meta);
uint32_t grid_bin_max_chunks();
uint32_t grid_bin_acc_bytes();
size_t grid_bin_workspace_bytes(const GridMeta& meta, uint32_t n);
void grid_backward_binned(hipStream_t stream, const GridMeta& meta, const GridMeta* dev_meta, uint32_t n, MatView x, const void* dL_dy, uint32_t dy_stride_sample,
                          uint32_t dy_stride_level, void* grad, bool accumulate, void* workspace,
                          uint32_t* fallback_count = nullptr);
void grid_backward_input(hipStream_t stream, const GridMeta& meta, bool fp32, uint32_t n, const void* dL_dy, uint32_t dy_stride, const float* dy_dx, MatViewMut dL_dx);
void grid_backward_backward_input(hipStream_t stream, const GridMeta& meta, const GridMeta* dev_meta, bool fp32, bool fp32_grad, uint32_t n, MatView x, MatView dL_ddLdx, const void* dL_dy,
                                  uint32_t dy_stride, const void* grid, const float* dy_dx, void* grad, void* dL_ddLdy, MatViewMut* dL_dx);

void oneblob_forward(hipStream_t stream, bool fp32, uint32_t n, uint32_t n_dims, uint32_t n_bins, MatView x, void* out, uint32_t out_stride);
void oneblob_backward_input(hipStream_t stream, bool fp32, uint32_t n, uint32_t n_dims, uint32_t n_bins, MatView x, const void* dL_dy, uint32_t dy_stride, MatViewMut dL_dx);
void identity_forward(hipStream_t stream, bool fp32, uint32_t n, uint32_t n_dims, float scale, float offset, MatView x, void* out, uint32_t out_stride);
void identity_backward_input(hipStream_t stream, bool fp32, uint32_t n, uint32_t n_dims, float scale, const void* dL_dy, uint32_t dy_stride, MatViewMut dL_dx);
void identity_backward_backward_input(hipStream_t stream, bool fp32, uint32_t n, uint32_t n_dims, float scale, MatView dL_ddLdx, void* dL_ddLdy, uint32_t dy_stride);
void periodic_forward(hipStream_t stream, bool triangle, bool fp32, uint32_t n, uint32_t n_dims, uint32_t n_frequencies, MatView x, void* out, uint32_t out_stride, float* dy_dx);
void periodic_backward_input(hipStream_t stream, bool fp32, uint32_t n, uint32_t n_dims, uint32_t outputs_per_input, const void* dL_dy, uint32_t dy_stride, const float* dy_dx, MatViewMut dL_dx);
void periodic_backward_backward_input(hipStream_t stream, bool triangle, bool fp32, uint32_t n, uint32_t n_dims, uint32_t n_frequencies, MatView x, MatView dL_ddLdx, const void* dL_dy,
                                       void* dL_ddLdy, uint32_t dy_stride, MatViewMut* dL_dx);
void composite_reduce_forward(hipStream_t stream, bool fp32, bool product, size_t n_elems, uint32_t n_nested, const void* in, void* out);
void composite_reduce_backward(hipStream_t stream, bool fp32, bool product, size_t n_elems, uint32_t n_nested, const void* in, const void* dL_dout, void* dL_din);
void composite_reduce_backward_backward(hipStream_t stream, bool fp32, size_t n_elems, uint32_t n_nested, const void* in, const void* tangents, const void* dL_dout, void* dL_ddLdout, void* q);
void sh_forward(hipStream_t stream, bool fp32, uint32_t n, uint32_t degree, MatView x, void* out, uint32_t out_stride);
void sh_backward_input(hipStream_t stream, bool fp32, uint32_t n, uint32_t degree, MatView x, const void* dL_dy, uint32_t dy_stride, MatViewMut dL_dx);
void sh_backward_backward_input(hipStream_t stream, bool fp32, uint32_t n, uint32_t degree, MatView x, MatView dL_ddLdx, const void* dL_dy, void* dL_ddLdy, uint32_t dy_stride, MatViewMut* dL_dx);

struct MlpLayer {
	uint32_t rows, cols;
	uint32_t w_off;
	uint32_t fwd_off;
	uint32_t bwd_off;
	uint32_t ks_fwd;
	uint32_t ks_bwd;
	uint32_t natural_k;
};

struct MlpDesc {
	uint32_t in_width, width, out_width, n_hidden, n_layers;
	uint32_t activation, output_activation;
	uint32_t n_frags_fwd, n_frags_bwd;
	uint32_t n_frags_r32;
	MlpLayer layers[MAX_MLP_LAYERS];
};

size_t mlp_image_bytes(const MlpDesc& d);
void mlp_prepare_weights(hipStream_t stream, const MlpDesc& d, const void* params, void* image, bool want_bwd);
void mlp_forward(hipStream_t stream, const MlpDesc& d, const void* image, uint32_t n, const void* x, void* out, void* hidden);
struct MlpIo {
	const void* x_half;
	uint32_t x_plane_features;
	MatView x_f32;
	uint32_t x_f32_dims;
	float x_scale, x_offset;
	uint32_t x_oneblob_bins;
	void* out_half;
	MatViewMut out_f32;
	uint32_t out_f32_dims;
};
void mlp_forward_io(hipStream_t stream, const MlpDesc& d, const void* image, uint32_t n, const MlpIo& io, void* hidden);
void mlp_backward(hipStream_t stream, const MlpDesc& d, const void* image, uint32_t n, const void* dL_dout, const void* out, const void* hidden, void* dhidden, void* dL_dx,
                  uint32_t dx_plane_features);
struct MlpTrainRequest {
	uint32_t n = 0;
	uint32_t x_plane_features = 0, oneblob_bins = 0, oneblob_dims = 0;
	uint32_t dims = 0;
	LossType loss = LossType::L2;
	bool external_dL_dy = false;
	bool data_pdf = false;
	bool out = false;
	bool dL_dx = false;
	uint32_t dx_plane_features = 0, dx_record_dims = 0;
	bool gradients = false;
	bool compact_context = false;
};
enum class MlpTrainKernel : uint32_t { None, R32ob, R32w, R32, R32a, Regs, Train };
struct MlpTrainPlan {
	bool ok = false;
	MlpTrainKernel kernel = MlpTrainKernel::None;
	const char* name = "";
	uint32_t grid = 0;
	MlpTrainRequest request;
	struct Config { int nb, nw, maxt; uint32_t lds_bytes, s; bool ok, image_in_lds, pw, regw; } config{};
	int regs_in_tiles = 0, regs_hidden = 0;
	bool regs_fast = false;
	bool r32ob_shared = false;
};
MlpTrainPlan mlp_train_plan(const MlpDesc& d, const MlpTrainRequest& request);
struct MlpTrainArgs {
	const void* image = nullptr;
	const void* x = nullptr;
	MatView oneblob_x{};
	const float *target = nullptr, *data_pdf = nullptr;
	const void* external_dL_dy = nullptr;
	float loss_scale = 1.0f;
	void *out = nullptr, *dL_dout = nullptr, *dL_dx = nullptr;
	float *L = nullptr, *slabs = nullptr;
	const float* dx_record_x = nullptr;
	uint32_t n_params = 0;
	const GridListTail* list_tail = nullptr;
};
bool mlp_train_item_map(const MlpTrainPlan& plan, GridItemMap& map);
void mlp_train_launch(hipStream_t stream, const MlpDesc& d, const MlpTrainPlan& plan, const MlpTrainArgs& args);
bool mlp_train_any_kernel(const MlpDesc& d, uint32_t n);
bool mlp_train_oneblob_in_kernel(const MlpDesc& d, uint32_t n, uint32_t n_bins);
bool mlp_train_compact_context(const MlpDesc& d, uint32_t n);
void mlp_expand_context(hipStream_t stream, uint32_t n, uint32_t dims, const void* compact_dL_dout, const float* compact_L, void* dL_dout, float* L);
struct AdamInReduce;
void mlp_reduce_slabs(hipStream_t stream, uint32_t n_params, uint32_t n_slabs, const float* slabs, void* grad_half, bool accumulate, const AdamInReduce* adam = nullptr);
void mlp_activation_backward_output(hipStream_t stream, uint32_t n_elems, uint32_t activation, const void* dL_dout, const void* out, void* result);
size_t wgrad_workspace_floats(uint32_t rows, uint32_t cols, uint32_t n);
struct WgradPanel { const void* dO; uint32_t ldo, rows; const void* In; uint32_t ldi, cols; void* grad; uint32_t ldg; bool dO_tiled, In_tiled; };
size_t wgrad_panels_workspace_floats(const WgradPanel* panels, uint32_t count, uint32_t n);
void mlp_wgrad_panels(hipStream_t stream, uint32_t n, const WgradPanel* panels, uint32_t count, bool accumulate, float* workspace);
void mlp_wgrad(hipStream_t stream, uint32_t n, const void* dO, uint32_t ldo, uint32_t rows, const void* In, uint32_t ldi, uint32_t cols,
               void* grad_half, uint32_t ldg, bool accumulate, float* workspace);
void mlp_layer_forward(hipStream_t stream, uint32_t n, const void* x, uint32_t ldx, const void* w, uint32_t rows, uint32_t cols, uint32_t activation, void* y, uint32_t ldy,
                       void* pre);
void mlp_layer_backward(hipStream_t stream, uint32_t n, const void* dL_dout, uint32_t ldo, const void* wt, uint32_t rows, uint32_t cols, uint32_t activation, const void* aux,
                        void* dL_din, uint32_t ldi);
void mlp_layer_transpose(hipStream_t stream, uint32_t rows, uint32_t cols, const void* w, void* wt);
void mlp_layer_tangent(hipStream_t stream, uint32_t n, const void* u_in, uint32_t ldu, const void* w, uint32_t rows, uint32_t cols, uint32_t activation, const void* aux, const void* g,
// ... 93 lines not shown
```

Before: 1.406 billion.

## Specialise hash-grid forward per level kind with buffer-descriptor loads

```diff
diff --git a/tiny-cuda-nn_amd/csrc/capi.cpp b/tiny-cuda-nn_amd/csrc/capi.cpp
--- a/tiny-cuda-nn_amd/csrc/capi.cpp
+++ b/tiny-cuda-nn_amd/csrc/capi.cpp
@@ -98,6 +98,7 @@
 	if (const char* e = getenv("TCNN_AMD_MLP_PRIO")) w.mlp_prio = (uint32_t)atoi(e);
 	w.listgrad_in_mlp = !env_is("TCNN_AMD_LISTGRAD_IN_MLP", '0');
 	w.mlp_layerwise = env_is("TCNN_AMD_MLP_LAYERWISE", '1');
+	w.fwd_kinds = !env_is("TCNN_AMD_FWD_KINDS", '0');
 	std::lock_guard<std::mutex> lock{g_switches_mutex};
 	g_switches = w;
 }
diff --git a/tiny-cuda-nn_amd/csrc/grid_device.h b/tiny-cuda-nn_amd/csrc/grid_device.h
--- a/tiny-cuda-nn_amd/csrc/grid_device.h
+++ b/tiny-cuda-nn_amd/csrc/grid_device.h
@@ -91,6 +91,40 @@
 	}
 }
 
+template <typename V, typename RS>
+__device__ inline V buffer_load_vec(const RS rs, const uint32_t voff) {
+	typedef uint32_t u4 __attribute__((ext_vector_type(4)));
+	static_assert(sizeof(V) == 4 || sizeof(V) == 8 || sizeof(V) == 16 || sizeof(V) == 32, "one or two buffer loads");
+	if constexpr (sizeof(V) == 4) return __builtin_bit_cast(V, __builtin_amdgcn_raw_buffer_load_b32(rs, voff, 0, 0));
+	else if constexpr (sizeof(V) == 8) return __builtin_bit_cast(V, __builtin_amdgcn_raw_buffer_load_b64(rs, voff, 0, 0));
+	else if constexpr (sizeof(V) == 16) return __builtin_bit_cast(V, __builtin_amdgcn_raw_buffer_load_b128(rs, voff, 0, 0));
+	else {
+		struct { u4 lo, hi; } t{__builtin_amdgcn_raw_buffer_load_b128(rs, voff, 0, 0), __builtin_amdgcn_raw_buffer_load_b128(rs, voff + 16u, 0, 0)};
+		return __builtin_bit_cast(V, t);
+	}
+}
+template <typename V, typename RS>
+__device__ inline void buffer_store_vec(const V v, const RS rs, const uint32_t voff) {
+	typedef uint32_t u2 __attribute__((ext_vector_type(2)));
+	typedef uint32_t u4 __attribute__((ext_vector_type(4)));
+	static_assert(sizeof(V) == 4 || sizeof(V) == 8 || sizeof(V) == 16, "one buffer store");
+	if constexpr (sizeof(V) == 4) __builtin_amdgcn_raw_buffer_store_b32(__builtin_bit_cast(uint32_t, v), rs, voff, 0, 0);
+	else if constexpr (sizeof(V) == 8) __builtin_amdgcn_raw_buffer_store_b64(__builtin_bit_cast(u2, v), rs, voff, 0, 0);
+	else __builtin_amdgcn_raw_buffer_store_b128(__builtin_bit_cast(u4, v), rs, voff, 0, 0);
+}
+template <int D, typename RS>
+__device__ inline void buffer_load_coords(const RS rs, const MatView& x, uint32_t i, float (&out)[D]) {
+	if (x.stride_dim == 1 && x.stride_sample == D && (D == 2 || D == 4)) {
+		typedef float vecD __attribute__((ext_vector_type(D)));
+		const vecD v = buffer_load_vec<vecD>(rs, i * (uint32_t)(D * 4));
+#pragma unroll
+		for (int d = 0; d < D; ++d) out[d] = v[d];
+	} else {
+#pragma unroll
+		for (int d = 0; d < D; ++d) out[d] = __builtin_bit_cast(float, __builtin_amdgcn_raw_buffer_load_b32(rs, i * x.stride_sample * 4u, d * x.stride_dim * 4u, 0));
+	}
+}
+
 __device__ inline uint32_t scatter_chunk(const GridLevel& lv, uint32_t index) {
 	return lv.scatter_shift != 0xffffffffu ? (index >> lv.scatter_shift) : (index / lv.scatter_per_chunk);
 }
diff --git a/tiny-cuda-nn_amd/csrc/k_grid_planes.hip b/tiny-cuda-nn_amd/csrc/k_grid_planes.hip
--- a/tiny-cuda-nn_amd/csrc/k_grid_planes.hip
+++ b/tiny-cuda-nn_amd/csrc/k_grid_planes.hip
@@ -18,23 +18,22 @@
 constexpr int FP_MAX_CHUNKS = GRID_FILTER_MAX_CHUNKS;
 constexpr int FP_PER_LANE = FP_MAX_CHUNKS / 64;
 
-template <int D, int F, int FP_SPT, bool LISTS>
-__global__ void __launch_bounds__(LISTS ? FP_LIST_THREADS : FP_THREADS) k_grid_fwd_planes(
-	const GridMeta* __restrict__ meta, const uint32_t* __restrict__ work, const uint32_t max_items, const uint32_t blocks_per_xcd, const uint32_t n, const MatView x,
-	const half_t* __restrict__ grid, half_t* __restrict__ out, unsigned long long* __restrict__ bits, const MlpPrepJob prep, const GridHitLists lists
-) {
+typedef uint32_t fp_u2 __attribute__((ext_vector_type(2)));
+typedef uint32_t fp_u4 __attribute__((ext_vector_type(4)));
+
+template <int D, int F, int FP_SPT, bool LISTS, GridFwdKind KIND>
+__device__ __forceinline__ void fwd_planes_item(const GridMeta* __restrict__ meta, const uint32_t w, const uint32_t level, const uint32_t n, const MatView& x, const half_t* __restrict__ grid,
+                                                half_t* __restrict__ out, unsigned long long* __restrict__ bits, const GridHitLists& lists, unsigned long long* lds_raw,
+                                                const uint32_t meta_interpolation, const uint32_t hash_type, const uint32_t (&primes)[D], const uint32_t tid, const uint32_t lane, const uint32_t wave) {
 	typedef typename VecOf<half_t, F>::type vecF;
+	constexpr bool FAST = KIND != GridFwdKind::Generic;
+	constexpr bool DENSE = KIND == GridFwdKind::Dense || KIND == GridFwdKind::DenseDiv;
+	constexpr bool DIV = KIND == GridFwdKind::DenseDiv;
 	constexpr int THREADS = LISTS ? FP_LIST_THREADS : FP_THREADS;
-	if (prep.image) {
-		const uint32_t total = (prep.desc.n_frags_fwd + prep.desc.n_frags_bwd + prep.desc.n_frags_r32) * 512;
-		for (uint32_t e = blockIdx.x * THREADS + threadIdx.x; e < total; e += gridDim.x * THREADS) mlp_prep_element(prep.desc, (const half_t*)prep.params, (half_t*)prep.image, e);
-	}
 	constexpr int FP_WAVE_SAMPLES = 64 * FP_SPT;
 	constexpr int FP_ITEM_SAMPLES = THREADS * FP_SPT;
 	constexpr int STAGE_ELEMS = FP_ITEM_SAMPLES << (D - 1);
 	constexpr int STAGE_U64 = STAGE_ELEMS * (int)GRID_HIT_WORDS / 2 + STAGE_ELEMS / 4;
-	static_assert(!LISTS || FP_ITEM_SAMPLES <= 65536, "16-bit sample numbers inside an item");
-	__shared__ __attribute__((aligned(16))) unsigned long long lds_raw[LISTS ? STAGE_U64 + 72 : (FP_THREADS / 64) * FP_SPT * FP_MAX_CHUNKS];
 	typedef unsigned long long plane_row[FP_SPT][FP_MAX_CHUNKS];
 	plane_row* planes = (plane_row*)lds_raw;
 	typedef __attribute__((address_space(3))) uint32_t lds_u32;
@@ -43,6 +42,357 @@
 	uint32_t* l_cnt = (uint32_t*)(lds_raw + STAGE_U64);
 	uint32_t* l_off = l_cnt + 64;
 	uint32_t* l_total = l_cnt + 128;
+	const uint32_t n_words = n / 64;
+	constexpr int C = 1 << D;
+	constexpr int R_ROWS = C / 2;
+	constexpr uint32_t HIT_SHIFT = grid_hit_mask_shift(D);
+	constexpr uint32_t ENTRY_BYTES = F * 2;
+	const uint32_t interpolation = FAST ? (uint32_t)InterpolationType::Linear : meta_interpolation;
+
+	uint32_t base = (w & 0xffffffu) * FP_ITEM_SAMPLES + wave * FP_WAVE_SAMPLES;
+	if constexpr (LISTS) base = grid_item_sample(lists.map, w & 0xffffffu, wave * FP_WAVE_SAMPLES);
+	if constexpr (!LISTS) { if (base >= n) return; }
+	const GridLevel lv = meta->levels[level];
+	const half_t* __restrict__ lgrid = grid + (size_t)lv.offset * F;
+	half_t* __restrict__ lout = out + (size_t)level * n * F;
+	const auto rs_grid = __builtin_amdgcn_make_buffer_rsrc((void*)lgrid, 0, FAST ? (int)(lv.size * ENTRY_BYTES) : 0, 0x00020000);
+	const auto rs_x = __builtin_amdgcn_make_buffer_rsrc((void*)x.data, 0, FAST ? (int)(((n - 1) * x.stride_sample + (D - 1) * x.stride_dim + 1) * 4u) : 0, 0x00020000);
+	const auto rs_out = __builtin_amdgcn_make_buffer_rsrc((void*)lout, 0, FAST ? (int)(n * ENTRY_BYTES) : 0, 0x00020000);
+	const uint32_t n_chunks = lv.scatter_n_chunks;
+	const bool want_bits = !LISTS && bits != nullptr && n_chunks > 1 && n_chunks <= FP_MAX_CHUNKS;
+	const bool lds_or = want_bits && n_chunks > 8;
+	const bool want_lists = LISTS && n_chunks > 1 && n_chunks <= FP_MAX_CHUNKS;
+	uint32_t cr[FP_SPT][R_ROWS];
+	uint32_t ipair[FP_SPT][R_ROWS];
+	const bool nearest = !FAST && interpolation == (uint32_t)InterpolationType::Nearest;
+	const uint32_t chunk_magic = DIV ? 0xffffffffu / lv.scatter_per_chunk : 0u;
+	auto chunk_of = [&](const uint32_t index) {
+		if constexpr (DIV) {
+			const uint32_t q = __umulhi(index, chunk_magic);
+			return q + (index - q * lv.scatter_per_chunk >= lv.scatter_per_chunk ? 1u : 0u);
+		} else if constexpr (FAST) return index >> lv.scatter_shift;
+		else return scatter_chunk(lv, index);
+	};
+	const uint32_t wrap_mask = lv.size_mask ? lv.size_mask : 0xffffffffu;
+
+	if (lds_or) {
+#pragma unroll
+		for (int k = 0; k < FP_SPT; ++k)
+#pragma unroll
+			for (int j = 0; j < FP_PER_LANE; ++j) planes[wave][k][lane + 64 * j] = 0ull;
+	}
+
+	constexpr int R = C / 2;
+	typedef typename VecOf<half_t, 2 * F>::type vecP __attribute__((aligned(2 * F)));
+	vecP P[FP_SPT][R];
+	vecF E[FP_SPT][R];
+	uint32_t sel[FP_SPT];
+	float pos[FP_SPT][D];
+	unsigned long long touched[FP_SPT];
+	auto note_chunk = [&](const int k, const uint32_t index) {
+		const uint32_t ch = chunk_of(index);
+		if (lds_or) {
+			__hip_atomic_fetch_or((__attribute__((address_space(3))) uint32_t*)&planes[wave][k][ch] + (lane >> 5), 1u << (lane & 31), __ATOMIC_RELAXED,
+			                      __HIP_MEMORY_SCOPE_WAVEFRONT);
+		} else {
+			touched[k] |= 1ull << ch;
+		}
+	};
+	float xall[FAST ? FP_SPT : 1][D];
+	if constexpr (FAST) {
+#pragma unroll
+		for (int k = 0; k < FP_SPT; ++k) buffer_load_coords<D>(rs_x, x, min(base + k * 64 + lane, n - 1), xall[k]);
+	}
+#pragma unroll
+	for (int k = 0; k < FP_SPT; ++k) {
+		const uint32_t i = min(base + k * 64 + lane, n - 1);
+		float xin[D];
+		if constexpr (FAST) {
+#pragma unroll
+			for (int d = 0; d < D; ++d) xin[d] = xall[k][d];
+		} else load_coords<D>(x, i, xin);
+		uint32_t cell[D];
+		float pd;
+#pragma unroll
+		for (int d = 0; d < D; ++d) cell[d] = pos_fract(xin[d], lv.scale, interpolation, &pos[k][d], &pd);
+		touched[k] = 0;
+		sel[k] = 0;
+		if constexpr (LISTS) {
+#pragma unroll
+			for (int r = 0; r < R_ROWS; ++r) { cr[k][r] = 0xffffffffu; ipair[k][r] = 0; }
+		}
+		const bool lists_here = LISTS && want_lists && base + k * 64 + lane < n;
+		uint32_t upper[D];
+		if constexpr (FAST) {
+#pragma unroll
+			for (int d = 1; d < D; ++d) upper[d] = cell[d] * (DENSE ? lv.stride[d] : primes[d]);
+		}
+#pragma unroll
+		for (int r = 0; r < R; ++r) {
+			if (r > 0 && nearest) { P[k][r] = P[k][0]; E[k][r] = E[k][0]; continue; }
+			uint32_t local[D];
+			local[0] = cell[0];
+#pragma unroll
+			for (int d = 1; d < D; ++d) local[d] = cell[d] + ((r >> (d - 1)) & 1);
+			uint32_t idx0, idx1;
+			if constexpr (DENSE) {
+				idx0 = cell[0];
+#pragma unroll
+				for (int d = 1; d < D; ++d) idx0 += upper[d] + (((r >> (d - 1)) & 1) ? lv.stride[d] : 0u);
+				idx0 &= wrap_mask;
+				idx1 = idx0 + 1u;
+				if (__builtin_expect(__ballot(idx0 >= lv.size - 1u) != 0ull, 0)) {
+					idx0 = level_index<D>(lv, primes, hash_type, local);
+					local[0] = cell[0] + 1;
+					idx1 = level_index<D>(lv, primes, hash_type, local);
+					const vecF lo = buffer_load_vec<vecF>(rs_grid, idx0 * ENTRY_BYTES), hi = buffer_load_vec<vecF>(rs_grid, idx1 * ENTRY_BYTES);
+					vecP p;
+#pragma unroll
+					for (int f = 0; f < F; ++f) { p[f] = lo[f]; p[F + f] = hi[f]; }
+					P[k][r] = p;
+				} else {
+					P[k][r] = buffer_load_vec<vecP>(rs_grid, idx0 * ENTRY_BYTES);
+				}
+			} else if constexpr (FAST) {
+				uint32_t h = 0;
+#pragma unroll
+				for (int d = 1; d < D; ++d) h ^= upper[d] + (((r >> (d - 1)) & 1) ? primes[d] : 0u);
+				idx0 = (cell[0] ^ h) & lv.size_mask;
+				idx1 = idx0 ^ ((cell[0] ^ (cell[0] + 1u)) & lv.size_mask);
+				const uint32_t a0 = idx0 & ~1u;
+				P[k][r] = buffer_load_vec<vecP>(rs_grid, a0 * ENTRY_BYTES);
+				const uint32_t d1 = idx1 - a0;
+				const bool own = d1 > 1u;
+				vecF e;
+#pragma unroll
+				for (int f = 0; f < F; ++f) e[f] = (half_t)0.0f;
+				if (own) e = buffer_load_vec<vecF>(rs_grid, idx1 * ENTRY_BYTES);
+				E[k][r] = e;
+				sel[k] |= ((idx0 - a0) | ((d1 & 1u) << 1) | (own ? 4u : 0u)) << (3 * r);
+			} else {
+				idx0 = level_index<D>(lv, primes, hash_type, local);
+				local[0] = cell[0] + 1;
+				idx1 = nearest ? idx0 : level_index<D>(lv, primes, hash_type, local);
+				const uint32_t a0 = lv.hashed ? (idx0 & ~1u) : min(idx0, lv.size - 2u);
+				P[k][r] = *(const vecP*)&lgrid[(size_t)a0 * F];
+				const uint32_t d1 = idx1 - a0;
+				const bool own = d1 > 1u;
+				vecF e;
+#pragma unroll
+				for (int f = 0; f < F; ++f) { if constexpr (F == 1) e = (half_t)0.0f; else e[f] = (half_t)0.0f; }
+				if (own) e = *(const vecF*)&lgrid[(size_t)idx1 * F];
+				E[k][r] = e;
+				sel[k] |= ((idx0 - a0) | ((d1 & 1u) << 1) | (own ? 4u : 0u)) << (3 * r);
+			}
+			if (want_bits) {
+				note_chunk(k, idx0);
+				if (!nearest) note_chunk(k, idx1);
+			}
+			if constexpr (LISTS) {
+				if (lists_here) {
+					const uint32_t ch_a = chunk_of(idx0), first = FAST && !DIV ? ch_a << lv.scatter_shift : ch_a * lv.scatter_per_chunk;
+					uint32_t rel_b = idx0 - first;
+					if (!nearest) {
+						const uint32_t ch_b = chunk_of(idx1);
+						if (ch_b == ch_a) rel_b = idx1 - first;
+						else {
+							const uint32_t at = atomicAdd(&lists.counts[level * GRID_HIT_COUNT_STRIDE], 1u);
+							if (at < lists.straggler_capacity) {
+								*(fp_u2*)&lists.stragglers[((size_t)level * lists.straggler_capacity + at) * 2] = fp_u2{i | (2u << (2 * r)) << HIT_SHIFT, ch_b};
+							}
+						}
+					}
+					ipair[k][r] = (idx0 - first) | rel_b << 16;
+					const uint32_t rank = __hip_atomic_fetch_add((lds_u32*)&l_cnt[ch_a], 1u, __ATOMIC_RELAXED, __HIP_MEMORY_SCOPE_WORKGROUP);
+					cr[k][r] = ch_a << 16 | rank;
+				}
+			}
+		}
+	}
+	if constexpr (LISTS) {
+		if (want_lists) {
+			__syncthreads();
+			if (wave == 0) {
+				const uint32_t cnt = l_cnt[lane];
+				l_cnt[lane] = 0;
+				uint32_t incl = cnt;
+#pragma unroll
+				for (int o = 1; o < 64; o <<= 1) {
+					const uint32_t up = __shfl_up(incl, o);
+					if (lane >= (uint32_t)o) incl += up;
+				}
+				l_off[lane] = incl - cnt;
+				uint32_t* heads = lists.heads + (size_t)level * GRID_HIT_HEADS * lists.n_items + (w & 0xffffffu);
+#ifdef TCNN_AMD_DEV
+				if (!(lists.dev_flags & 4u))
+#endif
+				{
+					if constexpr (FAST) {
+						const auto rs_h = __builtin_amdgcn_make_buffer_rsrc((void*)heads, 0, (int)((64u * lists.n_items + 1u) * 4u), 0x00020000);
+						__builtin_amdgcn_raw_buffer_store_b32(incl - cnt, rs_h, lane * lists.n_items * 4u, 0, 0);
+						if (lane == 63) __builtin_amdgcn_raw_buffer_store_b32(incl, rs_h, 64u * lists.n_items * 4u, 0, 0);
+					} else {
+						heads[(size_t)lane * lists.n_items] = incl - cnt;
+					}
+				}
+				if (lane == 63) { if constexpr (!FAST) heads[(size_t)64 * lists.n_items] = incl; *l_total = incl; }
+			}
+			__syncthreads();
+		}
+	}
+
+#pragma unroll
+	for (int k = 0; k < FP_SPT; ++k) {
+		const uint32_t i = base + k * 64 + lane;
+		vecF v[C];
+#pragma unroll
+		for (int r = 0; r < R; ++r) {
+			const uint32_t s = sel[k] >> (3 * r);
+			vecF lo, hi;
+#pragma unroll
+			for (int f = 0; f < F; ++f) { lo[f] = P[k][r][f]; hi[f] = P[k][r][F + f]; }
+			if constexpr (DENSE) {
+				v[2 * r] = lo;
+				v[2 * r + 1] = hi;
+			} else {
+				v[2 * r] = (s & 1u) ? hi : lo;
+				v[2 * r + 1] = (s & 4u) ? E[k][r] : ((s & 2u) ? hi : lo);
+			}
+		}
+		half_t acc[F];
+		half_t whs[C];
+#pragma unroll
+		for (int idx = 0; idx < C; ++idx) whs[idx] = (half_t)1.0f;
+		if (nearest) {
+#pragma unroll
+			for (int f = 0; f < F; ++f) acc[f] = v[0][f];
+		} else {
+#pragma unroll
+			for (int f = 0; f < F; ++f) acc[f] = (half_t)0.0f;
+#pragma unroll
+			for (int idx = 0; idx < C; ++idx) {
+				float weight = 1;
+#pragma unroll
+				for (int d = 0; d < D; ++d) weight *= (idx & (1 << d)) == 0 ? 1 - pos[k][d] : pos[k][d];
+				asm volatile("" : "+v"(weight));
+				const half_t wh = (half_t)weight;
+				whs[idx] = wh;
+#pragma unroll
+				for (int f = 0; f < F; ++f) {
+					half_t val;
+					val = v[idx][f];
+					acc[f] = __builtin_fmaf16(wh, val, acc[f]);
+				}
+			}
+		}
+		if (base + k * 64 < n) {
+			vecF o;
+#pragma unroll
+			for (int f = 0; f < F; ++f) { if constexpr (F == 1) o = acc[f]; else o[f] = acc[f]; }
+			if constexpr (FAST) buffer_store_vec<vecF>(o, rs_out, i * ENTRY_BYTES);
+			else *(vecF*)&lout[(size_t)i * F] = o;
+		}
+		if constexpr (LISTS) {
+			if (want_lists) {
+#pragma unroll
+				for (int r = 0; r < R_ROWS; ++r) {
+					const uint32_t v = cr[k][r];
+					if (v != 0xffffffffu) {
+						const uint32_t at = l_off[v >> 16] + (v & 0xffffu);
+						const uint32_t pr = ipair[k][r];
+						const bool no_b = (pr >> 16) == (pr & 0xffffu);
+						*(fp_u2*)(l_stage + at * GRID_HIT_WORDS) = fp_u2{pr, (uint32_t)__builtin_bit_cast(uint16_t, whs[2 * r]) | (no_b ? 0u : (uint32_t)__builtin_bit_cast(uint16_t, whs[2 * r + 1]) << 16)};
+						l_sidx[at] = (uint16_t)(wave * FP_WAVE_SAMPLES + k * 64 + lane);
+					}
+				}
+			}
+		}
+	}
+
+	if constexpr (LISTS) {
+		if (want_lists) {
+			__syncthreads();
+			const uint32_t total = *l_total, quads = (total * GRID_HIT_WORDS + 3) / 4, squads = (total + 7) / 8;
+			const size_t region = ((size_t)level * lists.n_items + (w & 0xffffffu)) * lists.item_capacity;
+			fp_u4* dst = (fp_u4*)(lists.elems + region * GRID_HIT_WORDS);
+			fp_u4* sdst = (fp_u4*)(lists.sidx + region);
+#ifdef TCNN_AMD_DEV
+			if (!(lists.dev_flags & 1u))
+#endif
+			{
+				bool through_descriptors = FAST;
+				int aux = 0;
+#ifdef TCNN_AMD_DEV
+				if (lists.dev_flags & 8u) through_descriptors = true, aux = 16;
+#endif
+				if (through_descriptors) {
+					const auto rs_e = __builtin_amdgcn_make_buffer_rsrc((void*)dst, 0, (int)(quads * 16u), 0x00020000);
+					const auto rs_s = __builtin_amdgcn_make_buffer_rsrc((void*)sdst, 0, (int)(squads * 16u), 0x00020000);
+					if (aux) {
+						for (uint32_t p = tid; p < quads; p += THREADS) __builtin_amdgcn_raw_buffer_store_b128(((const fp_u4*)l_stage)[p], rs_e, p * 16u, 0, 16);
+						for (uint32_t p = tid; p < squads; p += THREADS) __builtin_amdgcn_raw_buffer_store_b128(((const fp_u4*)l_sidx)[p], rs_s, p * 16u, 0, 16);
+					} else {
+						for (uint32_t p = tid; p < quads; p += THREADS) __builtin_amdgcn_raw_buffer_store_b128(((const fp_u4*)l_stage)[p], rs_e, p * 16u, 0, 0);
+						for (uint32_t p = tid; p < squads; p += THREADS) __builtin_amdgcn_raw_buffer_store_b128(((const fp_u4*)l_sidx)[p], rs_s, p * 16u, 0, 0);
+					}
+				} else {
+					for (uint32_t p = tid; p < quads; p += THREADS) dst[p] = ((const fp_u4*)l_stage)[p];
+					for (uint32_t p = tid; p < squads; p += THREADS) sdst[p] = ((const fp_u4*)l_sidx)[p];
+				}
+			}
+		}
+	}
+	if (want_bits) {
+#pragma unroll
+		for (int j = 0; j < FP_PER_LANE; ++j) {
+			if (j > 0 && !lds_or) break;
+			unsigned long long mine[FP_SPT];
+			const uint32_t ch = lane + 64 * j;
+			if (lds_or) {
+				__builtin_amdgcn_wave_barrier();
+#pragma unroll
+				for (int k = 0; k < FP_SPT; ++k) mine[k] = planes[wave][k][ch];
+			} else {
+#pragma unroll
+				for (int k = 0; k < FP_SPT; ++k) {
+					mine[k] = 0;
+					for (uint32_t c = 0; c < n_chunks; ++c) {
+						const unsigned long long b = __ballot((touched[k] >> c) & 1ull);
+						if (lane == c) mine[k] = b;
+					}
+				}
+			}
+			if (ch < n_chunks) {
+				unsigned long long* dst = bits + ((size_t)level * FP_MAX_CHUNKS + ch) * n_words + base / 64;
+				if (base + FP_WAVE_SAMPLES <= n) {
+					typedef unsigned long long u64x2 __attribute__((ext_vector_type(2)));
+#pragma unroll
+					for (int k = 0; k < FP_SPT; k += 2) *(u64x2*)&dst[k] = u64x2{mine[k], mine[k + 1]};
+				} else {
+#pragma unroll
+					for (int k = 0; k < FP_SPT; ++k) if (base + k * 64 < n) dst[k] = mine[k];
+				}
+			}
+		}
+	}
+}
+
+template <int D, int F, int FP_SPT, bool LISTS>
+__global__ void __launch_bounds__(LISTS ? FP_LIST_THREADS : FP_THREADS) k_grid_fwd_planes(
+	const GridMeta* __restrict__ meta, const uint32_t* __restrict__ work, const uint32_t max_items, const uint32_t blocks_per_xcd, const uint32_t n, const MatView x,
+	const half_t* __restrict__ grid, half_t* __restrict__ out, unsigned long long* __restrict__ bits, const MlpPrepJob prep, const GridHitLists lists, const uint32_t kinds_ok
+) {
+	constexpr int THREADS = LISTS ? FP_LIST_THREADS : FP_THREADS;
+	if (prep.image) {
+		const uint32_t total = (prep.desc.n_frags_fwd + prep.desc.n_frags_bwd + prep.desc.n_frags_r32) * 512;
+		for (uint32_t e = blockIdx.x * THREADS + threadIdx.x; e < total; e += gridDim.x * THREADS) mlp_prep_element(prep.desc, (const half_t*)prep.params, (half_t*)prep.image, e);
+	}
+	constexpr int FP_ITEM_SAMPLES = THREADS * FP_SPT;
+	constexpr int STAGE_ELEMS = FP_ITEM_SAMPLES << (D - 1);
+	constexpr int STAGE_U64 = STAGE_ELEMS * (int)GRID_HIT_WORDS / 2 + STAGE_ELEMS / 4;
+	static_assert(!LISTS || FP_ITEM_SAMPLES <= 65536, "16-bit sample numbers inside an item");
+	__shared__ __attribute__((aligned(16))) unsigned long long lds_raw[LISTS ? STAGE_U64 + 72 : (FP_THREADS / 64) * FP_SPT * FP_MAX_CHUNKS];
+	uint32_t* l_cnt = (uint32_t*)(lds_raw + STAGE_U64);
 	static_assert(FP_MAX_CHUNKS == 64, "one lane per chunk");
 	if constexpr (LISTS) {
 		if (threadIdx.x < 64) l_cnt[threadIdx.x] = 0;
@@ -58,282 +408,40 @@
 	const uint32_t xcd = blockIdx.x & 7u, slot = blockIdx.x >> 3;
 	const uint32_t n_items = work[xcd];
 	const uint32_t* __restrict__ items = work + 8 + (size_t)xcd * max_items;
+	const uint32_t* __restrict__ kinds = work + 8 + (size_t)8 * max_items;
 
 	const uint32_t interpolation = meta->interpolation;
 	const uint32_t hash_type = meta->hash_type;
 	uint32_t primes[D];
 #pragma unroll
 	for (int d = 0; d < D; ++d) primes[d] = meta->primes[d];
-	const uint32_t n_words = n / 64;
-	constexpr int C = 1 << D;
-	constexpr int R_ROWS = C / 2;
-	constexpr uint32_t HIT_SHIFT = grid_hit_mask_shift(D);
 
 	for (uint32_t it = slot; it < n_items; it += blocks_per_xcd) {
 		const uint32_t w = items[it];
 		const uint32_t level = w >> 24;
-		uint32_t base = (w & 0xffffffu) * FP_ITEM_SAMPLES + wave * FP_WAVE_SAMPLES;
-		if constexpr (LISTS) base = grid_item_sample(lists.map, w & 0xffffffu, wave * FP_WAVE_SAMPLES);
-		if constexpr (!LISTS) { if (base >= n) continue; }
-		const GridLevel lv = meta->levels[level];
-		const half_t* __restrict__ lgrid = grid + (size_t)lv.offset * F;
-		half_t* __restrict__ lout = out + (size_t)level * n * F;
-		const uint32_t n_chunks = lv.scatter_n_chunks;
-		const bool want_bits = !LISTS && bits != nullptr && n_chunks > 1 && n_chunks <= FP_MAX_CHUNKS;
-		const bool lds_or = want_bits && n_chunks > 8;
-		const bool want_lists = LISTS && n_chunks > 1 && n_chunks <= FP_MAX_CHUNKS;
-		uint32_t cr[FP_SPT][R_ROWS];
-		uint32_t ipair[FP_SPT][R_ROWS];
-		const bool nearest = interpolation == (uint32_t)InterpolationType::Nearest;
-
-		if (lds_or) {
-#pragma unroll
-			for (int k = 0; k < FP_SPT; ++k)
-#pragma unroll
-				for (int j = 0; j < FP_PER_LANE; ++j) planes[wave][k][lane + 64 * j] = 0ull;
-		}
-
-		constexpr int R = C / 2;
-		typedef typename VecOf<half_t, 2 * F>::type vecP __attribute__((aligned(2 * F)));
-		vecP P[FP_SPT][R];
-		vecF E[FP_SPT][R];
-		uint32_t sel[FP_SPT];
-		float pos[FP_SPT][D];
-		unsigned long long touched[FP_SPT];
-		auto note_chunk = [&](const int k, const uint32_t index) {
-			const uint32_t ch = scatter_chunk(lv, index);
-			if (lds_or) {
-				__hip_atomic_fetch_or((__attribute__((address_space(3))) uint32_t*)&planes[wave][k][ch] + (lane >> 5), 1u << (lane & 31), __ATOMIC_RELAXED,
-				                      __HIP_MEMORY_SCOPE_WAVEFRONT);
-			} else {
-				touched[k] |= 1ull << ch;
-			}
-		};
-#pragma unroll
-		for (int k = 0; k < FP_SPT; ++k) {
-			const uint32_t i = min(base + k * 64 + lane, n - 1);
-			float xin[D];
-			load_coords<D>(x, i, xin);
-			uint32_t cell[D];
-			float pd;
-#pragma unroll
-			for (int d = 0; d < D; ++d) cell[d] = pos_fract(xin[d], lv.scale, interpolation, &pos[k][d], &pd);
-			touched[k] = 0;
-			sel[k] = 0;
-			if constexpr (LISTS) {
-#pragma unroll
-				for (int r = 0; r < R_ROWS; ++r) { cr[k][r] = 0xffffffffu; ipair[k][r] = 0; }
-			}
-			const bool lists_here = LISTS && want_lists && base + k * 64 + lane < n;
-#pragma unroll
-			for (int r = 0; r < R; ++r) {
-				if (r > 0 && nearest) { P[k][r] = P[k][0]; E[k][r] = E[k][0]; continue; }
-				uint32_t local[D];
-				local[0] = cell[0];
-#pragma unroll
-				for (int d = 1; d < D; ++d) local[d] = cell[d] + ((r >> (d - 1)) & 1);
-				const uint32_t idx0 = level_index<D>(lv, primes, hash_type, local);
-				local[0] = cell[0] + 1;
-				const uint32_t idx1 = nearest ? idx0 : level_index<D>(lv, primes, hash_type, local);
-				const uint32_t a0 = lv.hashed ? (idx0 & ~1u) : min(idx0, lv.size - 2u);
-				P[k][r] = *(const vecP*)&lgrid[(size_t)a0 * F];
-				const uint32_t d1 = idx1 - a0;
-				const bool own = d1 > 1u;
-				vecF e;
-#pragma unroll
-				for (int f = 0; f < F; ++f) { if constexpr (F == 1) e = (half_t)0.0f; else e[f] = (half_t)0.0f; }
-				if (own) e = *(const vecF*)&lgrid[(size_t)idx1 * F];
-				E[k][r] = e;
-				sel[k] |= ((idx0 - a0) | ((d1 & 1u) << 1) | (own ? 4u : 0u)) << (3 * r);
-				if (want_bits) {
-					note_chunk(k, idx0);
-					if (!nearest) note_chunk(k, idx1);
-				}
-				if constexpr (LISTS) {
-					if (lists_here) {
-						const uint32_t ch_a = scatter_chunk(lv, idx0), first = ch_a * lv.scatter_per_chunk;
-						uint32_t rel_b = idx0 - first;
-						if (!nearest) {
-							const uint32_t ch_b = scatter_chunk(lv, idx1);
-							if (ch_b == ch_a) rel_b = idx1 - first;
-							else {
-								const uint32_t at = atomicAdd(&lists.counts[level * GRID_HIT_COUNT_STRIDE], 1u);
-								if (at < lists.straggler_capacity) {
-									typedef uint32_t u2 __attribute__((ext_vector_type(2)));
-									*(u2*)&lists.stragglers[((size_t)level * lists.straggler_capacity + at) * 2] = u2{i | (2u << (2 * r)) << HIT_SHIFT, ch_b};
-								}
-							}
-						}
-						ipair[k][r] = (idx0 - first) | rel_b << 16;
-						const uint32_t rank = __hip_atomic_fetch_add((lds_u32*)&l_cnt[ch_a], 1u, __ATOMIC_RELAXED, __HIP_MEMORY_SCOPE_WORKGROUP);
-						cr[k][r] = ch_a << 16 | rank;
-					}
-				}
-			}
-		}
-		if constexpr (LISTS) {
-			if (want_lists) {
-				__syncthreads();
-				if (wave == 0) {
-					const uint32_t cnt = l_cnt[lane];
-					l_cnt[lane] = 0;
-					uint32_t incl = cnt;
-#pragma unroll
-					for (int o = 1; o < 64; o <<= 1) {
-						const uint32_t up = __shfl_up(incl, o);
-						if (lane >= (uint32_t)o) incl += up;
-					}
-					l_off[lane] = incl - cnt;
-					uint32_t* heads = lists.heads + (size_t)level * GRID_HIT_HEADS * lists.n_items + (w & 0xffffffu);
-#ifdef TCNN_AMD_DEV
-					if (!(lists.dev_flags & 4u))
-#endif
-					heads[(size_t)lane * lists.n_items] = incl - cnt;
-					if (lane == 63) { heads[(size_t)64 * lists.n_items] = incl; *l_total = incl; }
-				}
-				__syncthreads();
-			}
-		}
-
-#pragma unroll
-		for (int k = 0; k < FP_SPT; ++k) {
-			const uint32_t i = base + k * 64 + lane;
-			vecF v[C];
-#pragma unroll
-			for (int r = 0; r < R; ++r) {
-				const uint32_t s = sel[k] >> (3 * r);
-				vecF lo, hi;
-#pragma unroll
-				for (int f = 0; f < F; ++f) { lo[f] = P[k][r][f]; hi[f] = P[k][r][F + f]; }
-				v[2 * r] = (s & 1u) ? hi : lo;
-				v[2 * r + 1] = (s & 4u) ? E[k][r] : ((s & 2u) ? hi : lo);
-			}
-			half_t acc[F];
-			half_t whs[C];
-#pragma unroll
-			for (int idx = 0; idx < C; ++idx) whs[idx] = (half_t)1.0f;
-			if (nearest) {
-#pragma unroll
-				for (int f = 0; f < F; ++f) acc[f] = v[0][f];
-			} else {
-#pragma unroll
-				for (int f = 0; f < F; ++f) acc[f] = (half_t)0.0f;
-#pragma unroll
-				for (int idx = 0; idx < C; ++idx) {
-					float weight = 1;
-#pragma unroll
-					for (int d = 0; d < D; ++d) weight *= (idx & (1 << d)) == 0 ? 1 - pos[k][d] : pos[k][d];
-					asm volatile("" : "+v"(weight));
-					const half_t wh = (half_t)weight;
-					whs[idx] = wh;
-#pragma unroll
-					for (int f = 0; f < F; ++f) {
-						half_t val;
-						val = v[idx][f];
-						acc[f] = __builtin_fmaf16(wh, val, acc[f]);
-					}
-				}
-			}
-			if (base + k * 64 < n) {
-				vecF o;
-#pragma unroll
-				for (int f = 0; f < F; ++f) { if constexpr (F == 1) o = acc[f]; else o[f] = acc[f]; }
-				*(vecF*)&lout[(size_t)i * F] = o;
-			}
-			if constexpr (LISTS) {
-				if (want_lists) {
-#pragma unroll
-					for (int r = 0; r < R_ROWS; ++r) {
-						const uint32_t v = cr[k][r];
-						if (v != 0xffffffffu) {
-							const uint32_t at = l_off[v >> 16] + (v & 0xffffu);
-							typedef uint32_t u2 __attribute__((ext_vector_type(2)));
-							const uint32_t pr = ipair[k][r];
-							const bool no_b = (pr >> 16) == (pr & 0xffffu);
-							*(u2*)(l_stage + at * GRID_HIT_WORDS) = u2{pr, (uint32_t)__builtin_bit_cast(uint16_t, whs[2 * r]) | (no_b ? 0u : (uint32_t)__builtin_bit_cast(uint16_t, whs[2 * r + 1]) << 16)};
-							l_sidx[at] = (uint16_t)(wave * FP_WAVE_SAMPLES + k * 64 + lane);
-						}
-					}
-				}
-			}
-		}
-
-		if constexpr (LISTS) {
-			if (want_lists) {
-				__syncthreads();
-				typedef uint32_t u4 __attribute__((ext_vector_type(4)));
-				const uint32_t total = *l_total, quads = (total * GRID_HIT_WORDS + 3) / 4, squads = (total + 7) / 8;
-				const size_t region = ((size_t)level * lists.n_items + (w & 0xffffffu)) * lists.item_capacity;
-				u4* dst = (u4*)(lists.elems + region * GRID_HIT_WORDS);
-				u4* sdst = (u4*)(lists.sidx + region);
-#ifdef TCNN_AMD_DEV
-				if (!(lists.dev_flags & 1u))
-#endif
-				{
-#ifdef TCNN_AMD_DEV
-					if (lists.dev_flags & 8u) {
-						const auto rs_e = __builtin_amdgcn_make_buffer_rsrc((void*)dst, 0, (int)(quads * 16u), 0x00020000);
-						const auto rs_s = __builtin_amdgcn_make_buffer_rsrc((void*)sdst, 0, (int)(squads * 16u), 0x00020000);
-						for (uint32_t p = tid; p < quads; p += THREADS) __builtin_amdgcn_raw_buffer_store_b128(((const u4*)l_stage)[p], rs_e, p * 16u, 0, 16);
-						for (uint32_t p = tid; p < squads; p += THREADS) __builtin_amdgcn_raw_buffer_store_b128(((const u4*)l_sidx)[p], rs_s, p * 16u, 0, 16);
-					} else
-#endif
-					{
-					for (uint32_t p = tid; p < quads; p += THREADS) dst[p] = ((const u4*)l_stage)[p];
-					for (uint32_t p = tid; p < squads; p += THREADS) sdst[p] = ((const u4*)l_sidx)[p];
-					}
-				}
-			}
-		}
-		if (want_bits) {
-#pragma unroll
-			for (int j = 0; j < FP_PER_LANE; ++j) {
-				if (j > 0 && !lds_or) break;
-				unsigned long long mine[FP_SPT];
-				const uint32_t ch = lane + 64 * j;
-				if (lds_or) {
-					__builtin_amdgcn_wave_barrier();
-#pragma unroll
-					for (int k = 0; k < FP_SPT; ++k) mine[k] = planes[wave][k][ch];
-				} else {
-#pragma unroll
-					for (int k = 0; k < FP_SPT; ++k) {
-						mine[k] = 0;
-						for (uint32_t c = 0; c < n_chunks; ++c) {
-							const unsigned long long b = __ballot((touched[k] >> c) & 1ull);
-							if (lane == c) mine[k] = b;
-						}
-					}
-				}
-				if (ch < n_chunks) {
-					unsigned long long* dst = bits + ((size_t)level * FP_MAX_CHUNKS + ch) * n_words + base / 64;
-					if (base + FP_WAVE_SAMPLES <= n) {
-						typedef unsigned long long u64x2 __attribute__((ext_vector_type(2)));
-#pragma unroll
-						for (int k = 0; k < FP_SPT; k += 2) *(u64x2*)&dst[k] = u64x2{mine[k], mine[k + 1]};
-					} else {
-#pragma unroll
-						for (int k = 0; k < FP_SPT; ++k) if (base + k * 64 < n) dst[k] = mine[k];
-					}
-				}
-			}
-		}
+		const uint32_t kind = kinds_ok ? kinds[level] : (uint32_t)GridFwdKind::Generic;
+#define TCNN_FWD_ITEM(KIND) fwd_planes_item<D, F, FP_SPT, LISTS, KIND>(meta, w, level, n, x, grid, out, bits, lists, lds_raw, interpolation, hash_type, primes, tid, lane, wave)
+		if (kind == (uint32_t)GridFwdKind::Dense) TCNN_FWD_ITEM(GridFwdKind::Dense);
+		else if (kind == (uint32_t)GridFwdKind::HashedPow2) TCNN_FWD_ITEM(GridFwdKind::HashedPow2);
+		else if (kind == (uint32_t)GridFwdKind::DenseDiv) TCNN_FWD_ITEM(GridFwdKind::DenseDiv);
+		else TCNN_FWD_ITEM(GridFwdKind::Generic);
+#undef TCNN_FWD_ITEM
 	}
 }
 
 template <int D, int F, int SPT>
 void launch_planes(hipStream_t s, const GridMeta* dm, const uint32_t* work, uint32_t max_items, uint32_t blocks_per_xcd, uint32_t n, MatView x, const void* grid, void* out, uint64_t* bits,
-                   const MlpPrepJob* prep_job, const GridHitLists* hit_lists) {
+                   const MlpPrepJob* prep_job, const GridHitLists* hit_lists, uint32_t kinds_ok) {
 	MlpPrepJob prep{};
 	if (prep_job) prep = *prep_job;
 	if (hit_lists) {
 		if constexpr (SPT == 8) throw std::runtime_error{"grid_forward_planes: hit lists come from the 2- and 4-samples-per-thread shapes"};
 		else
 		hipLaunchKernelGGL((k_grid_fwd_planes<D, F, SPT, true>), dim3(8 * blocks_per_xcd), dim3(FP_LIST_THREADS), 0, s, dm, work, max_items, blocks_per_xcd, n, x, (const half_t*)grid, (half_t*)out,
-		                   nullptr, prep, *hit_lists);
+		                   nullptr, prep, *hit_lists, kinds_ok);
 	} else {
 		hipLaunchKernelGGL((k_grid_fwd_planes<D, F, SPT, false>), dim3(8 * blocks_per_xcd), dim3(FP_THREADS), 0, s, dm, work, max_items, blocks_per_xcd, n, x, (const half_t*)grid, (half_t*)out,
-		                   (unsigned long long*)bits, prep, GridHitLists{});
+		                   (unsigned long long*)bits, prep, GridHitLists{}, kinds_ok);
 	}
 	HIP_CHECK_THROW(hipGetLastError());
 }
@@ -366,7 +474,7 @@
 	       div_round_up(n, FP_THREADS * grid_planes_spt(meta)) < (1u << 24);
 }
 
-void grid_planes_plan(const GridMeta& meta, uint32_t n, bool hit_lists, std::vector<uint32_t>& work, uint32_t& max_items, uint32_t& blocks_per_xcd) {
+void grid_planes_plan(const GridMeta& meta, uint32_t n, bool hit_lists, bool level_kinds, std::vector<uint32_t>& work, uint32_t& max_items, uint32_t& blocks_per_xcd) {
 	const uint32_t threads = hit_lists ? FP_LIST_THREADS : FP_THREADS;
 	const uint32_t items_per_level = div_round_up(n, threads * grid_planes_spt(meta));
 	float coarse_cost = 0.6f;
@@ -424,6 +532,7 @@
 		work[b] = (uint32_t)runs[b].size();
 		std::copy(runs[b].begin(), runs[b].end(), work.begin() + 8 + (size_t)b * max_items);
 	}
+	for (uint32_t l = 0; l < meta.n_levels; ++l) work.push_back((uint32_t)(level_kinds && !is_wide(l) ? grid_forward_level_kind(meta, l) : GridFwdKind::Generic));
 	blocks_per_xcd = std::max(1u, std::min(256u * FP_THREADS / threads, max_items));
 #ifdef TCNN_AMD_DEV
 	if (const char* e = getenv("TCNN_AMD_FWD_BLOCKS_PER_XCD")) blocks_per_xcd = std::max(1, atoi(e));
@@ -442,11 +551,14 @@
 		CHECK_THROW(m.n_windows == 1 || (n % hit_lists->item_samples == 0 && m.stride == hit_lists->n_items * m.window));
 	}
 	const uint32_t F = meta.n_features_per_level;
+	bool small = ((uint64_t)(n - 1) * x.stride_sample + (uint64_t)(meta.n_pos_dims - 1) * x.stride_dim + 1) * 4 < (1ull << 31) && (uint64_t)n * F * 2 < (1ull << 31);
+	if (hit_lists) small = small && (uint64_t)GRID_HIT_HEADS * hit_lists->n_items * 4 < (1ull << 31) && (uint64_t)hit_lists->item_capacity * GRID_HIT_WORDS * 4 < (1ull << 31);
+	const uint32_t kinds_ok = small ? 1u : 0u;
 #define TCNN_PLANES_F(D, SPT) \
 	switch (F) { \
-		case 2: return launch_planes<D, 2, SPT>(stream, dev_meta, dev_work, max_items, blocks_per_xcd, n, x, grid, out_planes, chunk_bits, prep_job, hit_lists); \
-		case 4: return launch_planes<D, 4, SPT>(stream, dev_meta, dev_work, max_items, blocks_per_xcd, n, x, grid, out_planes, chunk_bits, prep_job, hit_lists); \
-		default: return launch_planes<D, 8, SPT>(stream, dev_meta, dev_work, max_items, blocks_per_xcd, n, x, grid, out_planes, chunk_bits, prep_job, hit_lists); \
+		case 2: return launch_planes<D, 2, SPT>(stream, dev_meta, dev_work, max_items, blocks_per_xcd, n, x, grid, out_planes, chunk_bits, prep_job, hit_lists, kinds_ok); \
+		case 4: return launch_planes<D, 4, SPT>(stream, dev_meta, dev_work, max_items, blocks_per_xcd, n, x, grid, out_planes, chunk_bits, prep_job, hit_lists, kinds_ok); \
+		default: return launch_planes<D, 8, SPT>(stream, dev_meta, dev_work, max_items, blocks_per_xcd, n, x, grid, out_planes, chunk_bits, prep_job, hit_lists, kinds_ok); \
 	}
 #define TCNN_PLANES(D) \
 	if (grid_planes_spt(meta) == 8) { TCNN_PLANES_F(D, 8) } else if (grid_planes_spt(meta) == 4) { TCNN_PLANES_F(D, 4) } else { TCNN_PLANES_F(D, 2) }
diff --git a/tiny-cuda-nn_amd/csrc/model.h b/tiny-cuda-nn_amd/csrc/model.h
--- a/tiny-cuda-nn_amd/csrc/model.h
+++ b/tiny-cuda-nn_amd/csrc/model.h
@@ -424,12 +424,13 @@
 		uint32_t max_items = 0, blocks_per_xcd = 0;
 	};
 	PlanesPlan& planes_plan(uint32_t n_, bool hit_lists) {
-		const uint32_t n = n_ | (hit_lists ? 0x80000000u : 0u);
+		const bool level_kinds = switches().fwd_kinds;
+		const uint32_t n = n_ | (hit_lists ? 0x80000000u : 0u) | (level_kinds ? 0x40000000u : 0u);
 		auto it = m_planes_plans.find(n);
 		if (it != m_planes_plans.end()) return *it->second;
 		auto plan = std::make_unique<PlanesPlan>();
 		std::vector<uint32_t> work;
-		grid_planes_plan(m_meta, n_, hit_lists, work, plan->max_items, plan->blocks_per_xcd);
+		grid_planes_plan(m_meta, n_, hit_lists, level_kinds, work, plan->max_items, plan->blocks_per_xcd);
 		plan->dev_work.resize(work.size() * sizeof(uint32_t));
 		HIP_CHECK_THROW(hipMemcpy(plan->dev_work.data(), work.data(), work.size() * sizeof(uint32_t), hipMemcpyHostToDevice));
 		return *(m_planes_plans[n] = std::move(plan));
diff --git a/tiny-cuda-nn_amd/csrc/tcnn_common.h b/tiny-cuda-nn_amd/csrc/tcnn_common.h
--- a/tiny-cuda-nn_amd/csrc/tcnn_common.h
+++ b/tiny-cuda-nn_amd/csrc/tcnn_common.h
@@ -55,6 +55,7 @@
 	uint32_t mlp_prio = 1;
 	bool listgrad_in_mlp = true;
 	bool mlp_layerwise = false;
+	bool fwd_kinds = true;
 };
 Switches switches();
 void switches_reload();
@@ -102,7 +103,20 @@
 void grid_planes_to_rows(hipStream_t stream, const GridMeta& meta, uint32_t n, uint32_t width, const void* planes, void* rows, uint32_t row_stride);
 void grid_rows_to_planes(hipStream_t stream, const GridMeta& meta, uint32_t n, uint32_t width, const void* rows, uint32_t row_stride, void* planes);
 uint32_t grid_planes_spt(const GridMeta& meta);
-void grid_planes_plan(const GridMeta& meta, uint32_t n, bool hit_lists, std::vector<uint32_t>& work, uint32_t& max_items, uint32_t& blocks_per_xcd);
+enum class GridFwdKind : uint32_t { Generic = 0, Dense = 1, HashedPow2 = 2, DenseDiv = 3 };
+inline GridFwdKind grid_forward_level_kind(const GridMeta& meta, uint32_t level) {
+	const GridLevel& lv = meta.levels[level];
+	if (meta.interpolation != (uint32_t)InterpolationType::Linear || meta.grid_type != (uint32_t)GridType::Hash) return GridFwdKind::Generic;
+	if ((uint64_t)lv.size * meta.n_features_per_level * 2 >= (1ull << 31) || lv.size < 8) return GridFwdKind::Generic;
+	const bool records = lv.scatter_n_chunks > 1 && lv.scatter_n_chunks <= 64;
+	const bool by_shift = lv.scatter_shift < 32 && lv.scatter_per_chunk == (1u << lv.scatter_shift);
+	if (records && !by_shift && lv.scatter_per_chunk == 0) return GridFwdKind::Generic;
+	if (!lv.hashed) return lv.stride[0] != 1 ? GridFwdKind::Generic : (records && !by_shift ? GridFwdKind::DenseDiv : GridFwdKind::Dense);
+	if (records && !by_shift) return GridFwdKind::Generic;
+	if (meta.hash_type == (uint32_t)HashType::Rng || meta.primes[0] != 1 || lv.size_mask == 0 || lv.size_mask != lv.size - 1) return GridFwdKind::Generic;
+	return GridFwdKind::HashedPow2;
+}
+void grid_planes_plan(const GridMeta& meta, uint32_t n, bool hit_lists, bool level_kinds, std::vector<uint32_t>& work, uint32_t& max_items, uint32_t& blocks_per_xcd);
 struct MlpPrepJob;
 inline constexpr uint32_t grid_hit_mask_shift(uint32_t n_pos_dims) { return 32u - (1u << n_pos_dims); }
 constexpr uint32_t GRID_HIT_COUNT_STRIDE = 64;
```

New measurement: 1.420 billion (median of 6 runs). 1.01x the previous value.
